# PacificBiosciences/pb-StarPhase

Hardware: AMD Instinct MI355X
Metric: HiFi reads/sec diplotyped (HLA+CYP2D6) (higher is better)
Workload: dtype int32; 1 GPU; BASELINE configs[1] + configs[2] as ONE sample per step: HLA-A/-B 10000 HiFi reads vs IMGT/HLA v0.14.1 (11,199 DNA alleles) + CYP2D6 2000 targeted reads (39 templates), the six configs[2] scenarios in turn; a new sample uploaded every step; reads -> diplotypes; hla_reads=10000, cyp2d6_reads=2000, cyp2d6_lanes=6, hla_lanes=2, cyp2d6_consensus=launch pairs

## Files before the change

### pb-starphase_amd/csrc/sp_api.hip

```cpp
#include "sp_internal.h"
#include <algorithm>
#include <thread>
#include <atomic>
#include <cstring>
#include <new>
#include <unistd.h>

extern "C" {

int32_t sp_abi_version(void) { return SP_ABI_VERSION; }

int32_t sp_device_count(int32_t* count) {
    int n = 0;
    hipError_t e = hipGetDeviceCount(&n);
    if (count) *count = (e == hipSuccess) ? n : 0;
    return e == hipSuccess ? SP_OK : SP_ERR_NO_DEVICE;
}

int32_t sp_ctx_create(int32_t device, void* stream, sp_ctx** out) {
    if (!out) return SP_ERR_INVALID_ARG;
    *out = nullptr;
    static std::atomic<int> effective{-1};
    bool by_library = false;
    if (effective.load() < 0) {
        bool hip_up = false;
        char link[64];
        for (int fd = 0; fd < 1024 && !hip_up; ++fd) {
            char path[64]; std::snprintf(path, sizeof path, "/proc/self/fd/%d", fd);
            const ssize_t k = readlink(path, link, sizeof link - 1);
            if (k > 0) { link[k] = 0; hip_up = std::strcmp(link, "/dev/kfd") == 0; }
        }
        const char* had = std::getenv("GPU_MAX_HW_QUEUES");
        if (!had && !hip_up) { (void)setenv("GPU_MAX_HW_QUEUES", "16", 0); by_library = true; }
        const char* now = std::getenv("GPU_MAX_HW_QUEUES");
        effective.store(now ? std::atoi(now) : (hip_up ? 0 : 4));
    }
    const int hw_queues = effective.load() > 0 ? effective.load() : 4;
    int n = 0;
    if (hipGetDeviceCount(&n) != hipSuccess || n <= 0 || device < 0 || device >= n) return SP_ERR_NO_DEVICE;
    if (hipSetDevice(device) != hipSuccess) return SP_ERR_NO_DEVICE;
    hipDeviceProp_t prop;
    if (hipGetDeviceProperties(&prop, device) != hipSuccess) return SP_ERR_NO_DEVICE;
    if (std::strncmp(prop.gcnArchName, "gfx950", 6) != 0) return SP_ERR_NO_DEVICE;
    sp_ctx* ctx = new (std::nothrow) sp_ctx();
    if (!ctx) return SP_ERR_OUT_OF_MEMORY;
    ctx->device = device;
    ctx->num_cus = prop.multiProcessorCount > 0 ? prop.multiProcessorCount : 256;
    static bool set_here = false;
    if (by_library) set_here = true;
    ctx->hw_queues = hw_queues; ctx->hw_queues_by_library = set_here;
    ctx->hw_queues_effective = effective.load();
    { const char* kc = std::getenv("SP_K8_COMPOUND"); if (kc && *kc) ctx->k8_compound = std::atoi(kc); }
    { const char* ks = std::getenv("SP_K8_SIDE_ORDERS"); if (ks && *ks) ctx->k8_side_orders = std::max(0, std::min(3, std::atoi(ks))); }
    { const char* kp = std::getenv("SP_K8_PERSISTENT"); if (kp && *kp) ctx->k8_persistent = std::atoi(kp); }
    if (effective.load() == 0)
        ctx->warning = "the HIP runtime was initialised before the library's first context and GPU_MAX_HW_QUEUES was not set: the process's streams share the runtime's 4 hardware queues; "
                       "export GPU_MAX_HW_QUEUES=16 (or more) before the process initialises HIP";
    else if (hw_queues < 16)
        ctx->warning = "GPU_MAX_HW_QUEUES=" + std::to_string(hw_queues) + ": the library's streams share " + std::to_string(hw_queues) +
                       " hardware queues; export GPU_MAX_HW_QUEUES=16 (or more) before the process initialises HIP";
    if (stream) { ctx->stream = (hipStream_t)stream; ctx->own_stream = false; }
    else {
        if (hipStreamCreateWithFlags(&ctx->stream, hipStreamNonBlocking) != hipSuccess) { delete ctx; return SP_ERR_HIP; }
        ctx->own_stream = true;
    }
    if (hipEventCreate(&ctx->ev0) != hipSuccess || hipEventCreate(&ctx->ev1) != hipSuccess) { delete ctx; return SP_ERR_HIP; }
    *out = ctx;
    return SP_OK;
}

int32_t sp_ctx_get_info(const sp_ctx* ctx, sp_ctx_info* out) {
    if (!ctx || !out) return SP_ERR_INVALID_ARG;
    std::memset(out, 0, sizeof *out);
    out->device = ctx->device; out->num_cus = ctx->num_cus; out->hw_queues = ctx->hw_queues; out->hw_queues_set_by_library = ctx->hw_queues_by_library ? 1 : 0;
    std::snprintf(out->warning, sizeof out->warning, "%s", ctx->warning.c_str());
    return SP_OK;
}

static int32_t upload_finish(sp_seqset* s);
void sp_ctx_destroy(sp_ctx* ctx) {
    if (!ctx) return;
    for (sp_ctx*& h : ctx->helper) if (h) { sp_ctx_destroy(h); h = nullptr; }
    hipSetDevice(ctx->device);
    if (ctx->uploading) (void)upload_finish(ctx->uploading);
    if (ctx->copy_stream) { hipStreamSynchronize(ctx->copy_stream); hipStreamDestroy(ctx->copy_stream); ctx->copy_stream = nullptr; }
    if (ctx->ctl_stream) { hipStreamSynchronize(ctx->ctl_stream); hipStreamDestroy(ctx->ctl_stream); ctx->ctl_stream = nullptr; }
    if (ctx->ev_fork) hipEventDestroy(ctx->ev_fork);
    if (ctx->ev_join) hipEventDestroy(ctx->ev_join);
    hipStreamSynchronize(ctx->stream);
    for (sp_seqset* s : ctx->live_sets) {
        for (void* p : { (void*)s->d_words, (void*)s->d_nplane, (void*)s->d_word_off, (void*)s->d_len, (void*)s->d_kcode, (void*)s->d_kpos, (void*)s->d_koff }) if (p) ctx->dev_cap.erase(p);
        s->ctx = nullptr;
    }
    for (auto& kv : ctx->dev_cap) (void)hipFree(kv.first);
    if (ctx->scratch) hipFree(ctx->scratch);
    for (auto& kv : ctx->pool) if (kv.second.first) hipFree(kv.second.first);
    for (auto& kv : ctx->host_pool) if (kv.second.first) hipHostFree(kv.second.first);
    sp_profile_flush(ctx);
    for (hipEvent_t e : ctx->prof_free) hipEventDestroy(e);
    if (ctx->ev0) hipEventDestroy(ctx->ev0);
    if (ctx->ev1) hipEventDestroy(ctx->ev1);
    if (ctx->own_stream && ctx->stream) hipStreamDestroy(ctx->stream);
    delete ctx;
}

}
sp_ctx* sp_ctx_helper(sp_ctx* ctx, int i) {
    if (i < 0 || i > 6) return nullptr;
    if (!ctx->helper[i] && sp_ctx_create(ctx->device, nullptr, &ctx->helper[i]) != SP_OK) ctx->helper[i] = nullptr;
    if (ctx->helper[i]) { ctx->helper[i]->profiling = ctx->profiling; ctx->helper[i]->k5_block_pairs = ctx->k5_block_pairs; ctx->helper[i]->k8_persistent = ctx->k8_persistent; ctx->helper[i]->k8_side_orders = ctx->k8_side_orders; ctx->helper[i]->k8_compound = ctx->k8_compound; ctx->helper[i]->k8_side_max_blocks = ctx->k8_side_max_blocks; ctx->helper[i]->mm2_rescore = ctx->mm2_rescore; ctx->helper[i]->profile_rescore_counts = ctx->profile_rescore_counts; ctx->helper[i]->k1_best_n = ctx->k1_best_n; }
    return ctx->helper[i];
}
void sp_profile_merge(sp_ctx* into, sp_ctx* from) {
    sp_profile_flush(from);
    for (auto& kv : from->prof) { ProfileEntry& e = into->prof[kv.first]; e.ms += kv.second.ms; e.launches += kv.second.launches; e.cells += kv.second.cells; }
    from->prof.clear();
}
extern "C" {

int32_t sp_struct_size(const char* name) {
    if (!name) return -1;
#define SP_SZ(T) if (std::strcmp(name, #T) == 0) return (int32_t)sizeof(T);
    SP_SZ(sp_ctx_info)
    SP_SZ(sp_pair)
    SP_SZ(sp_aln)
    SP_SZ(sp_hla_db_desc)
    SP_SZ(sp_hla_realign)
    SP_SZ(sp_k1_seed_hit)
    SP_SZ(sp_hla_best)
    SP_SZ(sp_chain_problem)
    SP_SZ(sp_chain_result)
    SP_SZ(sp_region_hit)
    SP_SZ(sp_cyp_problem)
    SP_SZ(sp_cyp_call)
    SP_SZ(sp_cyp_locus)
    SP_SZ(sp_cyp_gene_def)
    SP_SZ(sp_cyp_config)
    SP_SZ(sp_cyp_db_stats)
    SP_SZ(sp_variant_problem)
    SP_SZ(sp_variant_result)
    SP_SZ(sp_sv_definitions)
    SP_SZ(sp_cons_config)
    SP_SZ(sp_cons_result)
    SP_SZ(sp_cons_problem)
    SP_SZ(sp_cons_output)
    SP_SZ(sp_priority_problem)
    SP_SZ(sp_priority_job)
    SP_SZ(sp_hla_call_config)
    SP_SZ(sp_hla_call)
    SP_SZ(sp_diplotype_settings)
    SP_SZ(sp_sample_inputs)
    SP_SZ(sp_starphase_timing)
    SP_SZ(sp_cyp_read_mapping)
    SP_SZ(sp_database_metadata)
    SP_SZ(sp_database_stats)
    SP_SZ(sp_gene_region)
    SP_SZ(sp_variant_detail)
    SP_SZ(sp_bam_read)
    SP_SZ(sp_affine_opts)
    SP_SZ(sp_affine_aln)
    SP_SZ(sp_k1_seed_info)
    SP_SZ(sp_cyp_region_variants)
    SP_SZ(sp_chain_build_info)
    SP_SZ(sp_variant_gene_stats)
    SP_SZ(sp_vcf_allele)
    SP_SZ(sp_vcf_deletion)
    SP_SZ(sp_mapping_stats)
    SP_SZ(sp_hla_rev_hit)
    SP_SZ(sp_batch_options)
    SP_SZ(sp_starphase_batch_timing)
    SP_SZ(sp_hla_alleles_stats)
    SP_SZ(sp_hla_cfg_mapping)
    SP_SZ(sp_hla_cfg_gene)
    SP_SZ(sp_pileup_col)
    SP_SZ(sp_support_summary)
    SP_SZ(sp_support_entry)
#undef SP_SZ
    return -1;
}

const char* sp_last_error(const sp_ctx* ctx) { return ctx ? ctx->err.c_str() : "null context"; }

int32_t sp_ctx_synchronize(sp_ctx* ctx) {
    if (!ctx) return SP_ERR_INVALID_ARG;
    SP_HIP_CHECK(ctx, hipStreamSynchronize(ctx->stream));
    return SP_OK;
}

int32_t sp_ctx_set_option(sp_ctx* ctx, const char* name, int64_t value) {
    if (!ctx || !name) return SP_ERR_INVALID_ARG;
    if (std::strcmp(name, "hla_split_genes") == 0) { ctx->split_genes = value != 0; return SP_OK; }
    if (std::strcmp(name, "k1_best_n") == 0) { if (value < 0 || value > 8) return sp_fail(ctx, SP_ERR_INVALID_ARG, "sp_ctx_set_option: k1_best_n is 0..8"); ctx->k1_best_n = (int)value; for (sp_ctx* h : ctx->helper) if (h) h->k1_best_n = ctx->k1_best_n; return SP_OK; }
    if (std::strcmp(name, "profile_rescore_counts") == 0) { ctx->profile_rescore_counts = value != 0; for (sp_ctx* h : ctx->helper) if (h) h->profile_rescore_counts = ctx->profile_rescore_counts; return SP_OK; }
    if (std::strcmp(name, "mm2_rescore") == 0) { ctx->mm2_rescore = (int)value; for (sp_ctx* h : ctx->helper) if (h) h->mm2_rescore = ctx->mm2_rescore; return SP_OK; }
    if (std::strcmp(name, "k8_side_orders") == 0) { if (value < 0 || value > 3) return sp_fail(ctx, SP_ERR_INVALID_ARG, "sp_ctx_set_option: k8_side_orders is 0 .. 3"); ctx->k8_side_orders = (int)value; for (sp_ctx* h : ctx->helper) if (h) h->k8_side_orders = ctx->k8_side_orders; return SP_OK; }
    if (std::strcmp(name, "k8_compound") == 0) { ctx->k8_compound = (int)value; for (sp_ctx* h : ctx->helper) if (h) h->k8_compound = ctx->k8_compound; return SP_OK; }
    if (std::strcmp(name, "k8_side_max_blocks") == 0) { if (value < 0) return sp_fail(ctx, SP_ERR_INVALID_ARG, "sp_ctx_set_option: k8_side_max_blocks >= 0"); ctx->k8_side_max_blocks = (int)value; for (sp_ctx* h : ctx->helper) if (h) h->k8_side_max_blocks = ctx->k8_side_max_blocks; return SP_OK; }
    if (std::strcmp(name, "k8_persistent") == 0) { if (value < 0 || value > 2) return sp_fail(ctx, SP_ERR_INVALID_ARG, "sp_ctx_set_option: k8_persistent is 0 (never), 1 (whenever a batch fits) or 2 (the library decides)"); ctx->k8_persistent = (int)value; ctx->k8_persist_backoff = 0; ctx->k8_persist_failures = 0; for (sp_ctx* h : ctx->helper) if (h) h->k8_persistent = ctx->k8_persistent; return SP_OK; }
    if (std::strcmp(name, "cons_retry_ladder") == 0) { ctx->cons_retry_ladder = value != 0; for (sp_ctx* h : ctx->helper) if (h) h->cons_retry_ladder = ctx->cons_retry_ladder; return SP_OK; }
    if (std::strcmp(name, "k5_block_pairs") == 0) { if (value < 0 || value > (1 << 20)) return sp_fail(ctx, SP_ERR_INVALID_ARG, "sp_ctx_set_option: k5_block_pairs is 0..1048576"); ctx->k5_block_pairs = (int)value; for (sp_ctx* h : ctx->helper) if (h) h->k5_block_pairs = ctx->k5_block_pairs; return SP_OK; }
    if (std::strcmp(name, "cyp_cohort_min_group") == 0) { if (value < 1 || value > 64) return sp_fail(ctx, SP_ERR_INVALID_ARG, "sp_ctx_set_option: cyp_cohort_min_group is 1..64"); ctx->cyp_cohort_min_group = (int)value; return SP_OK; }
    if (std::strcmp(name, "cyp_cohort_streams") == 0) { if (value < 1 || value > 8) return sp_fail(ctx, SP_ERR_INVALID_ARG, "sp_ctx_set_option: cyp_cohort_streams is 1..8"); ctx->cyp_cohort_streams = (int)value; return SP_OK; }
    if (std::strcmp(name, "hla_split_streams") == 0) { if (value < 1 || value > 4) return sp_fail(ctx, SP_ERR_INVALID_ARG, "sp_ctx_set_option: hla_split_streams is 1..4"); ctx->split_streams = (int)value; return SP_OK; }
    return sp_fail(ctx, SP_ERR_INVALID_ARG, std::string("sp_ctx_set_option: unknown option ") + name);
}

int32_t sp_profile_reset(sp_ctx* ctx) {
    if (!ctx) return SP_ERR_INVALID_ARG;
    for (sp_ctx* h : ctx->helper) if (h) sp_profile_reset(h);
    sp_profile_flush(ctx); ctx->prof.clear();
    unsigned long long* c = sp_counters(ctx);
    if (c) { hipSetDevice(ctx->device); hipMemsetAsync(c, 0, SPC_N * sizeof(unsigned long long), ctx->stream); }
    return SP_OK;
}

int32_t sp_profile_get(sp_ctx* ctx, const char* kernel, double* total_ms, uint64_t* launches, uint64_t* cells) {
    if (!ctx || !kernel) return SP_ERR_INVALID_ARG;
    sp_profile_flush(ctx);
    for (sp_ctx* h : ctx->helper) if (h) sp_profile_merge(ctx, h);
    static const struct { const char* name; int idx; } counters[] = {
        {"count:k1_cells_active", SPC_K1_ACTIVE}, {"count:k1_cells_executed", SPC_K1_EXECUTED}, {"count:k1_cells_resumed", SPC_K1_RESUMED},
        {"count:k1_cells_bytes", SPC_K1_BYTES}, {"count:cons_launches", SPC_CONS_LAUNCHES}, {"count:cons_columns", SPC_CONS_COLUMNS},
        {"count:dbg0", 6}, {"count:dbg1", 7}, {"count:dbg2", 8}, {"count:dbg3", 9}, {"count:dbg4", 10}, {"count:dbg5", 11}, {"count:dbg6", 12}, {"count:dbg7", 13} };
    for (const auto& c : counters) if (std::strcmp(kernel, c.name) == 0) {
        unsigned long long v = 0; unsigned long long* d = sp_counters(ctx);
        if (d) { hipSetDevice(ctx->device); if (hipMemcpyAsync(&v, d + c.idx, 8, hipMemcpyDeviceToHost, ctx->stream) != hipSuccess || hipStreamSynchronize(ctx->stream) != hipSuccess) return sp_fail(ctx, SP_ERR_HIP, "sp_profile_get: counter read failed"); }
        for (sp_ctx* h : ctx->helper) if (h) {
            unsigned long long hv = 0; unsigned long long* hd = sp_counters(h);
            if (hd && hipMemcpyAsync(&hv, hd + c.idx, 8, hipMemcpyDeviceToHost, h->stream) == hipSuccess && hipStreamSynchronize(h->stream) == hipSuccess) v += hv;
        }
        if (total_ms) *total_ms = 0.0;
        if (launches) *launches = 0;
        if (cells) *cells = v;
        return SP_OK;
    }
    if (std::strcmp(kernel, "pool:device") == 0) {
        uint64_t allocs = ctx->pool_allocs, bytes = ctx->scratch_bytes;
        for (const auto& b : ctx->pool) bytes += b.second.second;
        for (sp_ctx* h : ctx->helper) if (h) { allocs += h->pool_allocs; bytes += h->scratch_bytes; for (const auto& b : h->pool) bytes += b.second.second; }
        if (total_ms) *total_ms = 0.0;
        if (launches) *launches = allocs;
        if (cells) *cells = bytes;
        return SP_OK;
    }
    auto it = ctx->prof.find(kernel);
    ProfileEntry e; if (it != ctx->prof.end()) e = it->second;
    if (total_ms) *total_ms = e.ms;
    if (launches) *launches = e.launches;
    if (cells) *cells = e.cells;
    return SP_OK;
}


struct sp_upload {
    std::thread th;
    int32_t rc = SP_OK; std::string err;
    int format = SP_SEQ_ASCII;
    const uint8_t* src = nullptr; uint64_t src_bytes = 0;
    std::vector<uint64_t> rel;
    uint8_t* d_stage = nullptr; uint64_t* d_off = nullptr; uint32_t* d_flag = nullptr;
    uint8_t* ring = nullptr; size_t chunk = 0; int slots = 0;
    hipEvent_t slot_ev[4] = { nullptr, nullptr, nullptr, nullptr };
    size_t wbytes = 0;
};

static constexpr size_t UPLOAD_CHUNK = (size_t)8 << 20;
static constexpr int UPLOAD_SLOTS = 4;

static void upload_run(sp_seqset* s) {
    sp_upload* u = s->up; sp_ctx* ctx = s->ctx;
    hipStream_t st = ctx->copy_stream;
    auto bad = [&](hipError_t e, const char* what) { if (e != hipSuccess && u->rc == SP_OK) { u->rc = SP_ERR_HIP; u->err = std::string(what) + ": " + hipGetErrorString(e); } return e != hipSuccess; };
    if (bad(hipSetDevice(ctx->device), "hipSetDevice")) return;
    const uint32_t n = s->n;
    bad(hipMemcpyAsync(s->d_word_off, s->h_word_off.data(), ((size_t)n + 1) * sizeof(uint64_t), hipMemcpyHostToDevice, st), "offsets");
    if (n) bad(hipMemcpyAsync(s->d_len, s->h_len.data(), (size_t)n * sizeof(int32_t), hipMemcpyHostToDevice, st), "lengths");
    bad(hipMemsetAsync(s->d_words, 0, u->wbytes, st), "clear");
    if (u->src_bytes && u->rc == SP_OK) {
        bad(hipMemcpyAsync(u->d_off, u->rel.data(), ((size_t)n + 1) * 8, hipMemcpyHostToDevice, st), "staged offsets");
        bad(hipMemsetAsync(u->d_flag, 0, 4, st), "flag");
// ... 423 lines not shown
```

### pb-starphase_amd/csrc/sp_consensus.hip

```cpp
#include "sp_internal.h"
#include <atomic>
#include <cstdlib>
#include "sp_wfa.hip.h"
#include <algorithm>
#include <cstddef>
#include <cstring>
#include <map>
#include <string>

namespace {

constexpr int CB = 64;
constexpr int CH = 32;
#ifndef SP_K8_WAVES
#define SP_K8_WAVES 8
#endif
#ifndef SP_K8_MIN_WAVES
#define SP_K8_MIN_WAVES 4
#endif
constexpr int CWAVES = SP_K8_WAVES;
#ifndef SP_K8_DBG_READS
#define SP_K8_DBG_READS 16384
#endif
#define SP_K8_DBG_LAUNCHES (4194304 / SP_K8_DBG_READS)
#ifndef SP_K8_CW
#define SP_K8_CW 256
#endif
constexpr int CW = SP_K8_CW;
static_assert(CW % 64 == 0 && CW >= 64 && CW <= 512, "window length");
constexpr int CWIN = 512;
constexpr int RWORDS = (2 * CW + 320) / 16;
constexpr int NQ = 56;
constexpr int NWORK = 4;
constexpr int MAXKIDS = 16;
constexpr int CLUSTER = 64;
constexpr int RSLICES = 16;
constexpr int RGROUP = 16;
constexpr int QSV = 2 * (CW + 1) * 5, QSL = 2 * CW * 4, QE = QSV + QSL + 2 * (CW + 1);
enum { F_ACTIVE = 1, F_FINISHED = 2, F_LOST = 4 };
enum { M_NONE = 0, M_INIT = 1, M_WINDOW = 2, M_EXPAND = 3 };

struct CWork {
    int32_t mode, done;
    int32_t node, in_slot;
    int32_t T, n, replay;
    int32_t dual, split_at;
    int32_t go[2];
    int32_t n_kids, pad;
    int32_t pre_go[2];
    int32_t kid_node[MAXKIDS];
    int8_t  kid_base[MAXKIDS][2];
    int8_t  kid_split[MAXKIDS];
    uint8_t spec[2][CW];
};
struct CNode {
    int32_t used, id, complete;
    int32_t T, cur;
    int32_t dual, split_at, stopped[2], len[2];
    int32_t n, a, q;
    int16_t have_out, la_valid;
    int32_t wcap;
    long long cost0;
    long long rest;
    long long rest_out;
    uint32_t ev[2][5];
    int32_t pex_n, pex_L;
    int8_t  pex_kid[MAXKIDS];
    int32_t pad_head[2];
    int32_t dc[CW + 1];
    uint8_t spec[2][CW];
    int32_t pad_[3];
    __device__ __forceinline__ long long cost_at(int j) const { return cost0 + (long long)dc[j]; }
};
constexpr int NODE_HEAD_WORDS = 40, NODE_WORDS = (int)(sizeof(CNode) / 4), NODE_TAPE_WORDS = NODE_WORDS - NODE_HEAD_WORDS;
static_assert(offsetof(CNode, dc) == 4 * NODE_HEAD_WORDS && sizeof(CNode) % 16 == 0, "CNode layout");
struct CSearch {
    int32_t threshold, farthest, next_id, best_node, inflight, max_queue, per_size, wo_constraint;
    int32_t windows, cut_windows, expansions, pops_mod;
    long long pops, best_final;
    long long ticks[4];
    long long step_ticks, gap_ticks, last_end;
    int32_t compound, compound_ok;
    long long gap_ctl_ticks;
    int32_t steps, side_windows, side_expansions, adopted;
#ifdef SP_K8_PF_PROBE
    int32_t pf_win, pf_replay, pf_exp, pf_pad;
    unsigned long long idle_mask;
#endif
};
struct ConsMeta { int32_t e, c0, flags, pad; };
// ... 423 lines not shown
                }
                if (!__ballot(go && nm == 16 && left > 16)) break;
            }
        }, span, lane);
    } else if (span > 0 && !(d.flags & F_FINISHED) && !(et && rv.n <= span + CB)) {
        const int kk = lane - CH;
        dwfa_catchup_t(d, rv.n, [&]() {
            for (;;) {
                bool go = d.H >= 0 && d.H < rv.n && d.H + kk < span;
                if (go) { const int x = rbc(d.H); go = x < 4 && x == ca(d.c0 + d.H + kk); }
                if (!__ballot(go)) break;
                if (go) d.H += 1;
            }
        }, span, lane);
    } else {
        for (int Tl = 1; Tl <= span; ++Tl) {
            if (d.flags & (F_FINISHED | F_LOST)) break;
            dwfa_push_t(d, rv.n, rbc, [&](Dwfa& x, int Tc) {
                const int kk = lane - CH;
                for (;;) {
                    bool go = x.H >= 0 && x.H < rv.n && x.H + kk < Tc;
                    if (go) { const int b = rbc(x.H); go = b < 4 && b == ca(x.c0 + x.H + kk); }
                    if (!__ballot(go)) break;
                    if (go) x.H += 1;
                }
            }, Tl, ca(c0 + Tl - 1), et, lane);
        }
    }
    ACT_T(3);
    return d;
}

constexpr int KID_LA_KIDS = 4, KID_LA = CW / KID_LA_KIDS;
#ifndef SP_K8_KID_W0
#define SP_K8_KID_W0 32
#endif
constexpr int KID_W0 = SP_K8_KID_W0 < KID_LA ? SP_K8_KID_W0 : KID_LA;
#ifndef SP_K8_RAMP
#define SP_K8_RAMP 2
#endif
#ifndef SP_K8_KID_CALM
#define SP_K8_KID_CALM 6
#endif
constexpr int KID_CALM = SP_K8_KID_CALM;
struct UsedWords {
    int used, has_la, a_end, b_end, total;
    __device__ __forceinline__ UsedWords(int mode, int n, int n_kids) {
        used = mode == M_EXPAND ? n_kids : (mode == M_WINDOW ? n + 1 + n_kids : 1);
        has_la = mode != M_EXPAND || n_kids <= KID_LA_KIDS;
        a_end = 2 * used * 5; b_end = a_end + (has_la ? QSL : 0); total = b_end + 2 * used;
    }
    __device__ __forceinline__ int at(int c) const {
        if (c < a_end) { const int i = c / (used * 5), rem = c % (used * 5); return (i * (CW + 1) + rem / 5) * 5 + rem % 5; }
        if (c < b_end) return QSV + (c - a_end);
        const int r = c - b_end;
        return r < used ? QSV + QSL + r : QSV + QSL + (CW + 1) + (r - used);
    }
};
template <class BT> __device__ __forceinline__ uint32_t block_word(const BT& B, size_t blk, int o) {
    constexpr int EV = 2 * (CW + 1), EL = 2 * CW, EC = CW + 1;
    if (o < QSV) { const int e = o / 5, f = o % 5; return f < 4 ? (uint32_t)((B.PV[blk * EV + e] >> (16 * f)) & 0xFFFFull) : B.PE[blk * EV + e]; }
    if (o < QSV + QSL) { const int e = (o - QSV) / 4, f = (o - QSV) % 4; return (uint32_t)((B.PL[blk * EL + e] >> (16 * f)) & 0xFFFFull); }
    if (o < QSV + QSL + EC) return B.PC[blk * EC + (o - QSV - QSL)];
    return B.PR[blk * EC + (o - QSV - QSL - EC)];
}
#ifndef SP_K8_WRAMP0
#define SP_K8_WRAMP0 64
#endif
constexpr int WRAMP0 = SP_K8_WRAMP0;
constexpr int BULK_MARGIN_PLACED = 2;
constexpr int BULK_MARGIN = 8;
#ifndef SP_K8_AUTO_BATCHES
#define SP_K8_AUTO_BATCHES 1
#endif
constexpr int PERSIST_AUTO_BATCHES = SP_K8_AUTO_BATCHES;
#ifndef SP_K8_LIGHT
#define SP_K8_LIGHT 64
#endif
constexpr int PERSIST_LIGHT = SP_K8_LIGHT;
#ifndef SP_K8_DIRECT_BLOCKS
#define SP_K8_DIRECT_BLOCKS (680 * 8 / SP_K8_WAVES)
#endif
constexpr int DIRECT_BLOCKS = SP_K8_DIRECT_BLOCKS;
constexpr int32_t SP_K8_AGAIN = -777;
constexpr int PERSIST_BLOCKS = 128 * 8 / CWAVES;

template <int MAXP> __device__ __forceinline__ int block_problem(const ConsBatchT<MAXP>& B, int block) {
    int pi = 0;
    if constexpr (MAXP == 0) pi = B.block_prob[block];
    else {
#pragma unroll
        for (int i = 1; i < MAXP; ++i) if (i < B.n_prob && block >= B.p[i].first_block) pi = i;
    }
    return pi;
}
template <int MAXP> __device__ __forceinline__ int block_problem(const ConsBatchT<MAXP>& B) { return block_problem<MAXP>(B, (int)blockIdx.x); }

__device__ __forceinline__ size_t state_plane(int node, int slot, int cons) { return (size_t)((node * 2 + slot) * 2 + cons); }

__device__ __forceinline__ int read_cost(const Dwfa& a0, const Dwfa& a1, bool dualrun) {
    int c = -1;
    if (a0.flags & F_ACTIVE) c = a0.e;
    if (dualrun && (a1.flags & F_ACTIVE) && (c < 0 || a1.e < c)) c = a1.e;
    return c < 0 ? 0 : c;
}

template <int MAXP>
__device__ __forceinline__ void cons_step_body(const ConsBatchT<MAXP>& B, const int wrow) {
    __shared__ unsigned long long lv[2][CW + 1];
    __shared__ uint32_t le[2][CW + 1];
    __shared__ unsigned long long ll[2][CW];
    __shared__ uint32_t lc[CW + 1], lr[CW + 1];
    __shared__ uint8_t cwin[2][CWIN + CW];
    __shared__ uint32_t rwin[CWAVES][2][RWORDS + 2];
    __shared__ uint32_t cpk[2][(CWIN + CW) / 16 + 2];
    __shared__ ActScratch act[CWAVES];
    __shared__ CWork wk_s;
    const int pi = block_problem<MAXP>(B);
    const ConsParams P = B.p[pi];
    const bool coh = B.sync != nullptr;
    if (coh) {
        for (int x = threadIdx.x; x < (int)(sizeof(CWork) / 4); x += blockDim.x) ((uint32_t*)&wk_s)[x] = coh_load(((const uint32_t*)P.work) + x);
        __syncthreads();
    }
    const CWork* Wp = coh ? &wk_s : P.work + wrow;
    const int mode = Wp->mode;
    if (P.work->done || mode == M_NONE) return;
    if (wrow > 0 && P.n_blocks > DIRECT_BLOCKS) return;
    if (B.step_t && threadIdx.x == 0) atomicMin(&B.step_t[2 * pi], (unsigned long long)wall_clock64());
    const int lane = threadIdx.x & 63, wave = threadIdx.x >> 6;
    const int T = Wp->T, n = (mode == M_WINDOW || mode == M_EXPAND) ? Wp->n : 0;
    const int pre = mode == M_EXPAND ? n : 0;
    const int node = Wp->node, in_slot = Wp->in_slot;
    const int dual_in = Wp->dual, split_at = Wp->split_at;
    const int go0 = Wp->go[0], go1 = Wp->go[1];
    const int n_kids = (mode == M_EXPAND || mode == M_WINDOW) ? Wp->n_kids : 0;
    const uint8_t* Cn = P.C + (size_t)node * 2 * P.cs;
    for (int x = threadIdx.x; x < 2 * (CW + 1); x += blockDim.x) { (&lv[0][0])[x] = 0; (&le[0][0])[x] = 0; }
    for (int x = threadIdx.x; x < 2 * CW; x += blockDim.x) (&ll[0][0])[x] = 0;
    for (int x = threadIdx.x; x < CW + 1; x += blockDim.x) { lc[x] = 0; lr[x] = 0; }
    const int w0 = T - CWIN;
    for (int x = threadIdx.x; x < 2 * (CWIN + CW); x += blockDim.x) {
        const int i = x / (CWIN + CW), y = x % (CWIN + CW), pos = w0 + y;
        uint8_t v = 0;
        if (pos >= T) v = (pos - T < n) ? Wp->spec[dual_in ? i : 0][pos - T] : 0;
        else if (pos >= 0) v = coh_load((i == 1 && dual_in && pos >= split_at) ? &Cn[(size_t)P.cs + pos] : &Cn[pos]);
        cwin[i][y] = v;
    }
    __syncthreads();
    constexpr int CPW = (CWIN + CW) / 16 + 2;
    for (int x = threadIdx.x; x < 2 * CPW; x += blockDim.x) {
        const int i = x / CPW, w = x % CPW;
        uint32_t word = 0;
        for (int b = 0; b < 16; ++b) { const int y = w * 16 + b; if (y < CWIN + n) word |= (uint32_t)(cwin[i][y] & 3u) << (b << 1); }
        cpk[i][w] = word;
    }
    __syncthreads();
    const size_t plane = (size_t)B.total;
    for (int rr = 0; rr < P.rpw; ++rr) {
        const int r = (((int)blockIdx.x - P.first_block) * CWAVES + wave) * P.rpw + rr;
        if (r >= P.n) break;
        const size_t g = (size_t)P.first + r;
#ifdef SP_K8_TIMING
        const long long wt0 = wall_clock64();
        if (lane == 0) { act[wave].tk[0] = act[wave].tk[1] = act[wave].tk[2] = act[wave].tk[3] = 0; }
#endif
        const ReadInfo ri = B.info[g];
        ReadView rv; rv.w = ri.w; rv.np = ri.np; rv.n = ri.n;
        if (lane == 0) act[wave].staged = nullptr;
        Dwfa d0, d1;
        d0.H = SP_NEG; d0.e = 0; d0.c0 = 0; d0.flags = 0; d1 = d0;
        if (mode == M_INIT) {
            if (ri.off < 0) { d0.flags = F_ACTIVE | ((P.et && rv.n == 0) ? F_FINISHED : 0); d0.H = lane == CH ? 0 : SP_NEG; }
        } else {
            const size_t p0 = state_plane(node, in_slot, 0) * plane + g;
            const ConsMeta m0 = B.meta[p0];
            d0.H = h_load(B.H, p0 * CB + lane); d0.e = m0.e; d0.c0 = m0.c0; d0.flags = m0.flags;
            if (dual_in) {
                const size_t p1 = state_plane(node, in_slot, 1) * plane + g;
                const ConsMeta m1 = B.meta[p1];
                d1.H = h_load(B.H, p1 * CB + lane); d1.e = m1.e; d1.c0 = m1.c0; d1.flags = m1.flags;
            }
        }
        int rbase = 0;
        {
            int lo = 0x7FFFFFFF;
            if (d0.flags & F_ACTIVE) { const int x = T - d0.c0 - CB; lo = x < lo ? x : lo; }
            if (dual_in && (d1.flags & F_ACTIVE)) { const int x = T - d1.c0 - CB; lo = x < lo ? x : lo; }
            if (lo == 0x7FFFFFFF || lo < 0) lo = 0;
            rbase = (lo >> 4) << 4;
            const int w_first = rbase >> 4, w_last = (rv.n + 15) >> 4;
            if (lane < RWORDS + 2) {
                const int w = w_first + lane;
                rwin[wave][0][lane] = w <= w_last + 1 ? rv.w[w] : 0u;
                rwin[wave][1][lane] = (rv.np && w <= w_last + 1) ? rv.np[w] : 0u;
            }
            spw::wave_lds_sync();
        }
        auto rb = [&](int h) -> int {
            const int x = h - rbase;
            if ((unsigned)x < (unsigned)(RWORDS * 16)) {
                const uint32_t sh = (uint32_t)(x & 15) << 1;
                if ((rwin[wave][1][x >> 4] >> sh) & 1u) return 4;
                return (int)((rwin[wave][0][x >> 4] >> sh) & 3u);
            }
            return read_base(rv, h);
        };
        auto vote = [&](const Dwfa& a, const Dwfa& o, bool dualrun, int i, int col, int slot) {
            if (!(a.flags & F_ACTIVE) || (a.flags & (F_FINISHED | F_LOST))) return;
            if (dualrun && (o.flags & F_ACTIVE) && !(o.flags & F_LOST) && o.e < a.e) return;
            const int Tl = col - a.c0, k = lane - CH;
            const bool tip = a.H >= 0 && a.H + k == Tl;
            const int code = (tip && a.H < rv.n) ? rb(a.H) : 5;
            int dc = 0; unsigned long long word = 0;
#pragma unroll
            for (int b = 0; b < 4; ++b) { const bool s = __ballot(code == b) != 0; dc += s; word |= s ? (1ull << (16 * b)) : 0ull; }
            const bool ended = __ballot(tip) != 0 && __ballot(code == 4) == 0;
            if (lane == 0) {
                if (dc) atomicAdd(&lv[i][slot], word * vote_units(dc));
                else if (ended) atomicAdd(&le[i][slot], 12u);
            }
        };
        bool use_pk = mode == M_WINDOW;
        auto extender = [&](const ConsAccess& cacc, int i) {
            return [&cacc, i, &rb, wave, rbase, w0, lane, &use_pk, &rv](Dwfa& d, int Tc) {
                const int k = lane - CH;
                for (;;) {
                    int left = rv.n - d.H; { const int l2 = Tc - (d.H + k); left = l2 < left ? l2 : left; }
                    const bool go = d.H >= 0 && left > 0;
                    int nm = 0; bool more = false;
                    if (go) {
                        const int xr = d.H - rbase, yc = d.c0 + d.H + k - w0;
                        if (use_pk && xr >= 0 && xr < RWORDS * 16 && yc >= 0 && yc < CWIN + CW) {
                            const uint32_t a = __builtin_amdgcn_alignbit(rwin[wave][0][(xr >> 4) + 1], rwin[wave][0][xr >> 4], (uint32_t)(xr & 15) << 1);
                            const uint32_t nn = __builtin_amdgcn_alignbit(rwin[wave][1][(xr >> 4) + 1], rwin[wave][1][xr >> 4], (uint32_t)(xr & 15) << 1);
                            const uint32_t b = __builtin_amdgcn_alignbit(cpk[i][(yc >> 4) + 1], cpk[i][yc >> 4], (uint32_t)(yc & 15) << 1);
                            const uint32_t xo = a ^ b, mm = ((xo | (xo >> 1)) | nn) & 0x55555555u;
                            nm = mm ? (__builtin_ctz(mm) >> 1) : 16;
                            nm = nm < left ? nm : left;
                            more = nm == 16 && left > 16;
                        } else {
                            const int x = rb(d.H);
                            nm = (x < 4 && x == cacc.at(d.c0 + d.H + k)) ? 1 : 0;
// ... 288 lines not shown
                const int kb0 = Wp->kid_base[k][0], kb1 = Wp->kid_base[k][1], ksplit = Wp->kid_split[k];
                if (ksplit) e1 = e0;
                const bool kdual = dual_in || ksplit;
                ConsAccess k0 = ca0, k1 = ca1;
                k0.ov_pos = kb0 >= 0 ? TB : -1; k0.ov_base = kb0;
                k1.ov_pos = kb1 >= 0 ? TB : -1; k1.ov_base = kb1;
                if (ksplit) { k1.i = 0; }
                column(e0, e1, kdual, kb0 >= 0, kb1 >= 0, kb0, kb1, TB + 1, k0, k1);
                if (kb0 >= 0) vote(e0, e1, kdual, 0, TB + 1, s0 + k);
                if (kdual && kb1 >= 0) vote(e1, e0, kdual, 1, TB + 1, s0 + k);
                if (n_kids <= KID_LA_KIDS && (P.n < 256 || (r & 3) == 0)) {
#pragma unroll
                    for (int i = 0; i < 2; ++i) {
                        if (i == 1 && !kdual) continue;
                        if ((i ? kb1 : kb0) < 0) continue;
                        const Dwfa& a = i ? e1 : e0; const Dwfa& o = i ? e0 : e1;
                        if (!(a.flags & F_ACTIVE) || (a.flags & (F_FINISHED | F_LOST))) continue;
                        if (kdual && (o.flags & F_ACTIVE) && !(o.flags & F_LOST) && o.e < a.e) continue;
                        const int Tl = TB + 1 - a.c0, kd = lane - CH;
                        unsigned long long tips = __ballot(a.H >= 0 && a.H + kd == Tl && a.H < rv.n);
                        unsigned long long* const kl = &ll[0][0] + (size_t)(k * 2 + i) * KID_LA;
                        for (int cnt = 0; tips && cnt < 2; ++cnt) {
                            const int tl = __builtin_ctzll(tips); tips &= tips - 1;
                            const int h = __builtin_amdgcn_readlane(a.H, tl);
                            for (int x = lane; x < KID_LA - 1 && h + 1 + x < rv.n; x += SP_WAVE) {
                                const int b = rb(h + 1 + x);
                                if (b < 4) atomicAdd(&kl[x], 1ull << (16 * b));
                            }
                        }
                    }
                }
                const int grow = read_cost(e0, e1, kdual) - base_cost;
                const int len0 = kb0 >= 0 ? TB + 1 : (go0 ? TB : coh_load(&P.nodes[node].len[0]));
                const int len1 = kb1 >= 0 ? TB + 1 : (go1 ? TB : coh_load(&P.nodes[node].len[1]));
                const int extra = final_extra(e0, e1, kdual, len0, len1);
                if (lane == 0) { if (grow) atomicAdd(&lc[s0 + k], (uint32_t)grow); if (extra) atomicAdd(&lr[s0 + k], (uint32_t)extra); }
                const int kn = Wp->kid_node[k];
                store(e0, kn, 0, 0);
                if (kdual) store(e1, kn, 0, 1);
            }
            spw::wave_lds_sync();
        };
        if (mode == M_EXPAND) {
            if (pre > 0) { use_pk = true; win_pass(d0, d1, dual_in != 0, Wp->pre_go[0], Wp->pre_go[1], pre, true); use_pk = false; }
            expand_kids(d0, d1, T + pre, 0);
#ifdef SP_K8_DBG_PARTS
            if (B.dbg && lane == 0 && Wp->pad < SP_K8_DBG_LAUNCHES / 2 && g < SP_K8_DBG_READS) {
                const unsigned long long dt = (unsigned long long)(wall_clock64() - wt0);
                B.dbg[((size_t)Wp->pad * SP_K8_DBG_READS + g) * 2] = (dt > 0xFFFFFF ? 0xFFFFFFull : dt) | ((unsigned long long)(n_kids > 511 ? 511 : n_kids) << 24) | (3ull << 43) | ((unsigned long long)(pre > 511 ? 511 : pre) << 45);
                B.dbg[((size_t)Wp->pad * SP_K8_DBG_READS + g) * 2 + 1] = 0;
            }
#endif
            continue;
        }

        win_pass(d0, d1, dual_in != 0, go0, go1, n, false);
        if (n_kids > 0) {
            use_pk = false;
            if (lane == 0) act[wave].staged = nullptr;
            spw::wave_lds_sync();
            expand_kids(d0, d1, T + n, n + 1);
        }
    }
    __syncthreads();
    const UsedWords uw(mode, n, n_kids);
    if (P.n_blocks <= DIRECT_BLOCKS) {
        const size_t blk = (size_t)P.acc_block + (size_t)wrow;
        for (int x = threadIdx.x; x < 2 * uw.used; x += blockDim.x) {
            const int i = x / uw.used, e = i * (CW + 1) + x % uw.used;
            const unsigned long long v = (&lv[0][0])[e]; const uint32_t w = (&le[0][0])[e];
            if (v) atomicAdd(&B.PV[blk * 2 * (CW + 1) + e], v);
            if (w) atomicAdd(&B.PE[blk * 2 * (CW + 1) + e], w);
        }
        if (uw.has_la) for (int x = threadIdx.x; x < 2 * CW; x += blockDim.x) { const unsigned long long v = (&ll[0][0])[x]; if (v) atomicAdd(&B.PL[blk * 2 * CW + x], v); }
        for (int x = threadIdx.x; x < uw.used; x += blockDim.x) {
            if (lc[x]) atomicAdd(&B.PC[blk * (CW + 1) + x], lc[x]);
            if (lr[x]) atomicAdd(&B.PR[blk * (CW + 1) + x], lr[x]);
        }
        if (B.step_t && threadIdx.x == 0) atomicMax(&B.step_t[2 * pi + 1], (unsigned long long)wall_clock64());
        return;
    }
    for (int x = threadIdx.x; x < 2 * uw.used; x += blockDim.x) {
        const int i = x / uw.used, e = i * (CW + 1) + x % uw.used;
        B.PV[(size_t)blockIdx.x * 2 * (CW + 1) + e] = (&lv[0][0])[e];
        B.PE[(size_t)blockIdx.x * 2 * (CW + 1) + e] = (&le[0][0])[e];
    }
    if (uw.has_la) for (int x = threadIdx.x; x < 2 * CW; x += blockDim.x) B.PL[(size_t)blockIdx.x * 2 * CW + x] = (&ll[0][0])[x];
    for (int x = threadIdx.x; x < uw.used; x += blockDim.x) { B.PC[(size_t)blockIdx.x * (CW + 1) + x] = lc[x]; B.PR[(size_t)blockIdx.x * (CW + 1) + x] = lr[x]; }
    if (B.step_t && threadIdx.x == 0) atomicMax(&B.step_t[2 * pi + 1], (unsigned long long)wall_clock64());
}

template <int MAXP>
__global__ void __launch_bounds__(CWAVES * SP_WAVE, SP_K8_MIN_WAVES) cons_step_kernel(ConsBatchT<MAXP> B) { cons_step_body<MAXP>(B, (int)blockIdx.y); }
template <int MAXP>
__global__ void __launch_bounds__(CWAVES * SP_WAVE, 2) cons_step_wide_kernel(ConsBatchT<MAXP> B) { cons_step_body<MAXP>(B, (int)blockIdx.y); }

template <int MAXP>
__global__ void __launch_bounds__(512) cons_reduce_kernel(ConsBatchT<MAXP> B) {
    const int cluster = (int)blockIdx.x / RSLICES, slice = (int)blockIdx.x % RSLICES;
    int pi = 0;
    if constexpr (MAXP == 0) pi = B.cluster_prob[cluster];
    else {
#pragma unroll
        for (int i = 1; i < MAXP; ++i) if (i < B.n_prob && cluster >= B.p[i].first_cluster) pi = i;
    }
    const ConsParams P = B.p[pi];
    const int mode = P.work->mode;
    if (P.work->done || mode == M_NONE) return;
    const UsedWords uw(mode, mode == M_WINDOW ? P.work->n : 0, mode == M_EXPAND ? P.work->n_kids : 0);
    if (P.n_blocks <= DIRECT_BLOCKS) return;
    const int cl = cluster - P.first_cluster;
    const int members = P.n_blocks - cl * CLUSTER < CLUSTER ? P.n_blocks - cl * CLUSTER : CLUSTER;
    const size_t blk0 = (size_t)P.first_block + (size_t)cl * CLUSTER;
    constexpr int NG = CLUSTER / RGROUP;
    const int per = (uw.total + RSLICES - 1) / RSLICES;
    const int c_lo = slice * per, c_hi = c_lo + per < uw.total ? c_lo + per : uw.total;
    for (int idx = threadIdx.x; idx < (c_hi - c_lo) * NG; idx += blockDim.x) {
        const int o = uw.at(c_lo + idx / NG), m0 = (idx % NG) * RGROUP;
        uint32_t v[RGROUP];
#pragma unroll
        for (int m = 0; m < RGROUP; ++m) v[m] = m0 + m < members ? block_word(B, blk0 + m0 + m, o) : 0u;
        uint32_t sum = 0;
#pragma unroll
        for (int m = 0; m < RGROUP; ++m) sum += v[m];
#pragma unroll
        for (int d = 1; d < NG; d <<= 1) sum += __shfl_xor(sum, d);
        if (idx % NG == 0) B.Q[(size_t)cluster * QE + o] = sum;
    }
}

struct ColVotes { uint32_t w[4], end; };

__device__ __forceinline__ int col_candidates(const uint32_t* w5, int col, int cap, int et, int min_count, double min_af, int out[4]) {
    if (col >= cap) return 0;
    int order[4] = { 0, 1, 2, 3 };
#pragma unroll
    for (int a = 0; a < 4; ++a)
#pragma unroll
        for (int b = a + 1; b < 4; ++b) if (w5[order[b]] > w5[order[a]]) { const int t = order[a]; order[a] = order[b]; order[b] = t; }
    const uint32_t w1 = w5[order[0]], total = w5[0] + w5[1] + w5[2] + w5[3];
    const bool go = et ? w1 > 0 : (total > w5[4] && w1 > 0);
    if (!go) return 0;
    uint32_t need = 12u * (uint32_t)min_count; if (w1 < need) need = w1;
    int n = 0;
    out[n++] = order[0];
#pragma unroll
    for (int a = 1; a < 4; ++a) { const uint32_t w = w5[order[a]]; if (w > 0 && w >= need && (double)w >= min_af * (double)total) out[n++] = order[a]; }
    return n;
}

__device__ __forceinline__ int col_candidates_packed(const uint32_t* w5, int col, int cap, int et, int min_count, double min_af, uint32_t& packed) {
    packed = 0;
    if (col >= cap) return 0;
    uint32_t wa = w5[0], wb = w5[1], wc = w5[2], wd = w5[3]; uint32_t ca = 0, cb = 1, cc = 2, cd = 3;
#define SP_CSW(x, y, cx, cy) if (y > x) { const uint32_t tw_ = x; x = y; y = tw_; const uint32_t tc_ = cx; cx = cy; cy = tc_; }
    SP_CSW(wa, wb, ca, cb) SP_CSW(wa, wc, ca, cc) SP_CSW(wa, wd, ca, cd) SP_CSW(wb, wc, cb, cc) SP_CSW(wb, wd, cb, cd) SP_CSW(wc, wd, cc, cd)
#undef SP_CSW
    const uint32_t total = wa + wb + wc + wd;
    const bool go = et ? wa > 0 : (total > w5[4] && wa > 0);
    if (!go) return 0;
    uint32_t need = 12u * (uint32_t)min_count; if (wa < need) need = wa;
    int n = 1; packed = ca;
    const double floor_w = min_af * (double)total;
    if (wb > 0 && wb >= need && (double)wb >= floor_w) { packed |= cb << (2 * n); ++n; }
    if (wc > 0 && wc >= need && (double)wc >= floor_w) { packed |= cc << (2 * n); ++n; }
    if (wd > 0 && wd >= need && (double)wd >= floor_w) { packed |= cd << (2 * n); ++n; }
    return n;
}

template <int MAXP>
__device__ __forceinline__ void cons_control_body(const ConsBatchT<MAXP>& B) {
    extern __shared__ uint8_t proc[];
    __shared__ uint32_t acc[QE];
    uint32_t (*sv)[CW + 1][5] = reinterpret_cast<uint32_t (*)[CW + 1][5]>(acc);
    uint32_t (*sl)[CW][4] = reinterpret_cast<uint32_t (*)[CW][4]>(acc + QSV);
    uint32_t* sc = acc + QSV + QSL; uint32_t* sr = sc + (CW + 1);
    __shared__ CNode nh[NQ];
    __shared__ CWork wks[NWORK];
    __shared__ CSearch ss;
    __shared__ int copy_from[NWORK], copy_len[NWORK], need_la[NWORK], replay_of[NWORK];
    struct KidCopy { int from, T, n, nk, dual; int8_t node[4], b0[4], b1[4], sp[4]; uint8_t spec[2][CW]; };
    static_assert(KID_LA_KIDS <= 4, "KidCopy");
    __shared__ KidCopy kcopy[NWORK];
    const int pi = blockIdx.x;
    const ConsParams P = B.p[pi];
    const int tid = threadIdx.x;
    const bool coh = B.sync != nullptr;
    const int nside = (coh || P.n_blocks > DIRECT_BLOCKS) ? 0 : (B.nside < NWORK - 1 ? B.nside : NWORK - 1);
    const int n_orders = 1 + nside;
    CWork& wk = wks[0];
    const long long tk0 = wall_clock64();
    for (int x = tid; x < NQ * NODE_HEAD_WORDS; x += blockDim.x)
        ((uint32_t*)&nh[x / NODE_HEAD_WORDS])[x % NODE_HEAD_WORDS] = ((const uint32_t*)&P.nodes[x / NODE_HEAD_WORDS])[x % NODE_HEAD_WORDS];
    for (int x = tid; x < n_orders * (int)(sizeof(CWork) / 4); x += blockDim.x) ((uint32_t*)wks)[x] = ((const uint32_t*)P.work)[x];
    for (int x = tid; x < (int)(sizeof(CSearch) / 4); x += blockDim.x) ((uint32_t*)&ss)[x] = ((const uint32_t*)P.srch)[x];
    const int proc_words = (P.cap + 2 + 3) / 4;
    for (int x = tid; x < proc_words; x += blockDim.x) ((uint32_t*)proc)[x] = ((const uint32_t*)P.processed)[x];
    for (int x = tid; x < QE; x += blockDim.x) acc[x] = 0;
    if (tid < NWORK) { copy_from[tid] = -1; copy_len[tid] = 0; need_la[tid] = -1; replay_of[tid] = -1; kcopy[tid].nk = 0; if (tid >= n_orders) wks[tid].mode = M_NONE; }
    __syncthreads();
    if (wk.done) return;
    auto tape_word_used = [](const CNode& x, int w) {
        if (!x.used) return false;
        if (w == 0) return true;
        if (x.n <= 0) return false;
        if (w < CW + 1) return w <= x.n;
        const int sw = w - (CW + 1);
        return sw < 2 * (CW / 4) && (sw % (CW / 4)) * 4 < x.n;
    };
    for (int x = tid; x < NQ * NODE_TAPE_WORDS; x += blockDim.x) {
        const int k = x / NODE_TAPE_WORDS, w = x % NODE_TAPE_WORDS;
        if (tape_word_used(nh[k], w)) ((uint32_t*)&nh[k])[NODE_HEAD_WORDS + w] = ((const uint32_t*)&P.nodes[k])[NODE_HEAD_WORDS + w];
    }
    auto load_votes = [&](const int w) {
        const int mode_in = wks[w].mode, n_in = (mode_in == M_WINDOW || mode_in == M_EXPAND) ? wks[w].n : 0;
        if (mode_in == M_NONE) return;
        const UsedWords uw(mode_in, n_in, wks[w].n_kids);
        if (P.n_blocks <= DIRECT_BLOCKS) {
            const int u = uw.used, ev = 2 * u, el = uw.has_la ? 2 * CW : 0, E = ev + ev + el + u + u;
            const size_t blk = (size_t)P.acc_block + (size_t)w;
            for (int c = tid; c < E; c += blockDim.x) {
                if (c < ev || (c >= 2 * ev && c < 2 * ev + el)) {
                    const bool exact = c < ev;
                    const int e = exact ? (c / u) * (CW + 1) + c % u : c - 2 * ev;
                    unsigned long long* src = exact ? B.PV + blk * 2 * (CW + 1) + e : B.PL + blk * 2 * CW + e;
                    const unsigned long long sum = coh ? __hip_atomic_exchange(src, 0ull, __ATOMIC_RELAXED, __HIP_MEMORY_SCOPE_AGENT) : *src;
                    if (sum) {
                        if (!coh) *src = 0ull;
                        uint32_t* dst = exact ? acc + e * 5 : acc + QSV + e * 4;
#pragma unroll
                        for (int f = 0; f < 4; ++f) dst[f] = (uint32_t)((sum >> (16 * f)) & 0xFFFFull);
                    }
                } else {
                    uint32_t* src; uint32_t* dst;
                    if (c < 2 * ev) { const int cc = c - ev, e = (cc / u) * (CW + 1) + cc % u; src = B.PE + blk * 2 * (CW + 1) + e; dst = acc + e * 5 + 4; }
                    else if (c < 2 * ev + el + u) { const int e = c - 2 * ev - el; src = B.PC + blk * (CW + 1) + e; dst = acc + QSV + QSL + e; }
                    else { const int e = c - 2 * ev - el - u; src = B.PR + blk * (CW + 1) + e; dst = acc + QSV + QSL + (CW + 1) + e; }
                    const uint32_t sum = coh ? __hip_atomic_exchange(src, 0u, __ATOMIC_RELAXED, __HIP_MEMORY_SCOPE_AGENT) : *src;
                    if (sum) { if (!coh) *src = 0u; *dst = sum; }
                }
            }
        } else {
            const int parts = P.n_clusters;
            for (int c = tid; c < uw.total; c += blockDim.x) {
                const int o = uw.at(c);
                uint32_t sum = 0;
                for (int c0 = 0; c0 < parts; c0 += 8) {
                    uint32_t v[8];
#pragma unroll
                    for (int q = 0; q < 8; ++q) v[q] = c0 + q < parts ? B.Q[(size_t)(P.first_cluster + c0 + q) * QE + o] : 0u;
#pragma unroll
                    for (int q = 0; q < 8; ++q) sum += v[q];
                }
                acc[o] = sum;
            }
        }
    };
    const int lane = tid & (SP_WAVE - 1);
    auto cands = [&](const uint32_t* w5, int col, int out[4]) { return col_candidates(w5, col, P.cap, P.et, P.min_count, P.min_af, out); };
    auto node_free = [&](int k) {
        const int np = nh[k].pex_n;
        for (int j = 0; j < np; ++j) { CNode& c = nh[nh[k].pex_kid[j]]; c.used = 0; c.complete = 0; }
        nh[k].pex_n = 0; nh[k].used = 0; nh[k].complete = 0;
    };
    uint8_t* Cb = P.C;
    int la_fresh = -1;
    auto trim_queue = [&]() {
// ... 536 lines not shown
                if (lane == 0 && W.n == bcol) {
                    Plan fp; fp.nc0 = bn0; fp.nc1 = bn1; fp.cd0 = bc0; fp.cd1 = bc1;
                    const int kids = !W.dual ? bn0 + (P.allow_dual ? bn0 * (bn0 - 1) / 2 : 0) : (bn0 ? bn0 : 1) * (bn1 ? bn1 : 1);
                    unsigned long long fm = free_mask;
                    int made = 0;
                    for (int k = 0; k < kids && fm; ++k) {
                        int b0, b1, sp;
                        kid_of(fp, W.dual, k, b0, b1, sp);
                        const int kn = __builtin_ctzll(fm); fm &= fm - 1;
                        nh[kn].used = 2; nh[kn].complete = 0; nh[kn].pex_n = 0;
                        W.kid_node[made] = kn; W.kid_base[made][0] = (int8_t)b0; W.kid_base[made][1] = (int8_t)b1; W.kid_split[made] = (int8_t)sp;
                        ++made;
                    }
                    W.n_kids = made;
                    ss.compound += 1;
                }
                spw::wave_lds_sync();
            }
        }
    }
    __syncthreads();
    for (int w = 0; w < n_orders; ++w) {
        if (copy_from[w] < 0) continue;
        const CWork& W = wks[w];
        const int cfrom = copy_from[w], clen = copy_len[w];
        for (int k = 0; k < W.n_kids; ++k) {
            const int kn = W.kid_node[k];
            const bool split = W.kid_split[k] != 0;
            for (int i = 0; i < 2; ++i) {
                if (i == 1 && !(W.dual || split)) continue;
                const uint4* src = reinterpret_cast<const uint4*>(P.C + ((size_t)cfrom * 2 + ((i == 1 && split) ? 0 : i)) * P.cs);
                uint8_t* dst = P.C + ((size_t)kn * 2 + i) * P.cs;
                const int whole = clen >> 4, tail = clen & 15;
                for (int y = tid; y < whole + (tail ? 1 : 0); y += blockDim.x) {
                    uint4 v;
                    if (coh) {
                        const unsigned long long* s8 = reinterpret_cast<const unsigned long long*>(src + y);
                        const unsigned long long lo = coh_load(s8), hi = coh_load(s8 + 1);
                        v.x = (uint32_t)lo; v.y = (uint32_t)(lo >> 32); v.z = (uint32_t)hi; v.w = (uint32_t)(hi >> 32);
                    } else v = src[y];
                    if (y == whole && W.kid_base[k][i] >= 0) reinterpret_cast<uint8_t*>(&v)[tail] = (uint8_t)W.kid_base[k][i];
                    if (coh) {
                        unsigned long long* d8 = reinterpret_cast<unsigned long long*>(reinterpret_cast<uint4*>(dst) + y);
                        coh_store(d8, (unsigned long long)v.x | ((unsigned long long)v.y << 32)); coh_store(d8 + 1, (unsigned long long)v.z | ((unsigned long long)v.w << 32));
                    } else reinterpret_cast<uint4*>(dst)[y] = v;
                }
                if (tid == 0 && tail == 0 && W.kid_base[k][i] >= 0) put(&dst[clen], (uint8_t)W.kid_base[k][i], coh);
            }
        }
    }
    if (tid == 0) {
        const long long tk4 = wall_clock64(); ss.ticks[0] += tk1 - tk0; ss.ticks[1] += tk2 - tk1; ss.ticks[2] += tk3 - tk2; ss.ticks[3] += tk4 - tk3;
        if (B.step_t) {
            const long long st0 = (long long)coh_load(&B.step_t[2 * pi]), st1 = (long long)coh_load(&B.step_t[2 * pi + 1]);
            if (st1 > 0 && st0 <= st1) {
                ss.step_ticks += st1 - st0;
                if (ss.last_end > 0 && st0 >= ss.last_end) ss.gap_ticks += st0 - ss.last_end;
                if (tk0 >= st1) { ss.gap_ticks += tk0 - st1; ss.gap_ctl_ticks += tk0 - st1; }
            }
            put(&B.step_t[2 * pi], ~0ull, coh); put(&B.step_t[2 * pi + 1], 0ull, coh);
            ss.last_end = tk4;
        }
    }
#ifdef SP_K8_SEARCH_TICKS
    if (tid == 0) { ss.ticks[0] += 100 * ts_iters - (tk1 - tk0); ss.ticks[1] += ts_pick - (tk2 - tk1); ss.ticks[3] += ts_block - (wall_clock64() - tk3); }
#endif
    __syncthreads();
    for (int x = tid; x < NQ * NODE_HEAD_WORDS; x += blockDim.x)
        put(&((uint32_t*)&P.nodes[x / NODE_HEAD_WORDS])[x % NODE_HEAD_WORDS], ((const uint32_t*)&nh[x / NODE_HEAD_WORDS])[x % NODE_HEAD_WORDS], coh);
    for (int x = tid; x < NQ * NODE_TAPE_WORDS; x += blockDim.x) {
        const int k = x / NODE_TAPE_WORDS, w = x % NODE_TAPE_WORDS;
        if (tape_word_used(nh[k], w)) ((uint32_t*)&P.nodes[k])[NODE_HEAD_WORDS + w] = ((const uint32_t*)&nh[k])[NODE_HEAD_WORDS + w];
    }
    for (int x = tid; x < n_orders * (int)(sizeof(CWork) / 4); x += blockDim.x) put(&((uint32_t*)P.work)[x], ((const uint32_t*)wks)[x], coh);
    for (int x = tid; x < (int)(sizeof(CSearch) / 4); x += blockDim.x) ((uint32_t*)P.srch)[x] = ((const uint32_t*)&ss)[x];
    for (int x = tid; x < proc_words; x += blockDim.x) ((uint32_t*)P.processed)[x] = ((const uint32_t*)proc)[x];
    if (tid == 0 && B.prog) {
        __hip_atomic_store(B.prog + 2 * pi, (uint32_t)wk.pad, __ATOMIC_RELAXED, __HIP_MEMORY_SCOPE_SYSTEM);
        if (wk.done) __hip_atomic_store(B.prog + 2 * pi + 1, 1u, __ATOMIC_RELAXED, __HIP_MEMORY_SCOPE_SYSTEM);
    }
}

template <int MAXP>
__global__ void __launch_bounds__(1024) cons_control_kernel(ConsBatchT<MAXP> B) { cons_control_body<MAXP>(B); }

constexpr long long PERSIST_TIMEOUT = 400000000ll;
constexpr double PERSIST_READY_S = 0.5;
__device__ __forceinline__ bool persist_wait(const uint32_t* word, uint32_t at_least, uint32_t* abort_word) {
    const long long t0 = wall_clock64();
    for (uint32_t spins = 1;; ++spins) {
        if (__hip_atomic_load(word, __ATOMIC_RELAXED, __HIP_MEMORY_SCOPE_AGENT) >= at_least) return true;
        __builtin_amdgcn_s_sleep(1);
        if ((spins & 63u) == 0) {
            if (__hip_atomic_load(abort_word, __ATOMIC_RELAXED, __HIP_MEMORY_SCOPE_AGENT)) return false;
            if (wall_clock64() - t0 > PERSIST_TIMEOUT) { __hip_atomic_store(abort_word, 1u, __ATOMIC_RELAXED, __HIP_MEMORY_SCOPE_AGENT); return false; }
        }
    }
}

template <int MAXP>
__global__ void __launch_bounds__(CWAVES * SP_WAVE, SP_K8_MIN_WAVES) cons_step_persist_kernel(ConsBatchT<MAXP> B) {
    __shared__ int go_on;
    const int pi = block_problem<MAXP>(B);
    uint32_t* sy = B.sync + 4 * pi; uint32_t* abort_word = B.sync + 4 * B.n_prob;
    for (uint32_t k = 1;; ++k) {
        if (threadIdx.x == 0) go_on = persist_wait(sy + 0, k - 1, abort_word) ? 1 : 0;
        __syncthreads();
        if (!go_on) break;
        if (coh_load(&B.p[pi].work->done)) break;
        cons_step_body<MAXP>(B, 0);
        asm volatile("s_waitcnt vmcnt(0)" ::: "memory");
        __syncthreads();
        if (threadIdx.x == 0) __hip_atomic_fetch_add(sy + 1, 1u, __ATOMIC_RELAXED, __HIP_MEMORY_SCOPE_AGENT);
    }
}

template <int MAXP>
__global__ void __launch_bounds__(1024) cons_control_persist_kernel(ConsBatchT<MAXP> B) {
    __shared__ int go_on;
    const int pi = blockIdx.x;
    const uint32_t nb = (uint32_t)B.p[pi].n_blocks;
    uint32_t* sy = B.sync + 4 * pi; uint32_t* abort_word = B.sync + 4 * B.n_prob;
    if (threadIdx.x == 0 && B.ready) __hip_atomic_fetch_add(B.ready, 1u, __ATOMIC_RELAXED, __HIP_MEMORY_SCOPE_SYSTEM);
    for (uint32_t k = 1;; ++k) {
        if (threadIdx.x == 0) {
            go_on = persist_wait(sy + 1, nb * k, abort_word) ? 1 : 0;
            if (go_on && k > B.step_cap) { __hip_atomic_store(abort_word, 2u, __ATOMIC_RELAXED, __HIP_MEMORY_SCOPE_AGENT); go_on = 0; }
        }
        __syncthreads();
        if (!go_on) break;
        __builtin_amdgcn_fence(__ATOMIC_ACQUIRE, "agent");
        cons_control_body<MAXP>(B);
        asm volatile("s_waitcnt vmcnt(0)" ::: "memory");
        __syncthreads();
        const bool done = coh_load(&B.p[pi].work->done) != 0;
        if (threadIdx.x == 0) __hip_atomic_store(sy + 0, k, __ATOMIC_RELAXED, __HIP_MEMORY_SCOPE_AGENT);
        if (done) break;
    }
    if (threadIdx.x == 0 && B.prog) {
        const uint32_t ab = __hip_atomic_load(abort_word, __ATOMIC_RELAXED, __HIP_MEMORY_SCOPE_AGENT);
        if (ab) __hip_atomic_store(B.prog + 2 * pi + 1, 1u + ab, __ATOMIC_RELAXED, __HIP_MEMORY_SCOPE_SYSTEM);
    }
}

__global__ void cons_setup_kernel(ConsSetup S, ReadInfo* __restrict__ info) {
    const int r = blockIdx.x * blockDim.x + threadIdx.x;
    if (r >= S.n) return;
    const uint32_t rid = S.idx ? S.idx[r] : (uint32_t)r;
    ReadInfo ri;
    ri.w = S.reads.words + S.reads.word_off[rid];
    ri.np = S.reads.nplane ? S.reads.nplane + S.reads.word_off[rid] : nullptr;
    ri.n = S.reads.len[rid]; ri.off0 = S.offsets ? S.offsets[r] : -1; ri.off = ri.off0 < 0 ? -1 : ri.off0 + max(0, min(S.cmp_len, ri.n)); ri.pad = 0;
    info[S.first + r] = ri;
}

__global__ void cons_setup_many_kernel(const ConsSetup* __restrict__ S, int n_prob, int total, ReadInfo* __restrict__ info) {
    const int t = blockIdx.x * blockDim.x + threadIdx.x;
    if (t >= total) return;
    int lo = 0, hi = n_prob - 1;
    while (lo < hi) { const int mid = (lo + hi + 1) >> 1; if (S[mid].first <= t) lo = mid; else hi = mid - 1; }
    while (lo + 1 < n_prob && S[lo].n == 0 && S[lo + 1].first <= t) ++lo;
    const ConsSetup& q = S[lo];
    const int r = t - q.first;
    if (r < 0 || r >= q.n) return;
    const uint32_t rid = q.idx ? q.idx[r] : (uint32_t)r;
    ReadInfo ri;
    ri.w = q.reads.words + q.reads.word_off[rid];
    ri.np = q.reads.nplane ? q.reads.nplane + q.reads.word_off[rid] : nullptr;
    ri.n = q.reads.len[rid]; ri.off0 = q.offsets ? q.offsets[r] : -1; ri.off = ri.off0 < 0 ? -1 : ri.off0 + max(0, min(q.cmp_len, ri.n)); ri.pad = 0;
    info[t] = ri;
}

template <int MAXP>
__global__ void __launch_bounds__(SP_WAVE) cons_finalize_kernel(ConsBatchT<MAXP> B, uint8_t* is_cons1, int32_t* score1, int32_t* score2) {
    const int vblock = (int)blockIdx.x / CWAVES, wave = (int)blockIdx.x % CWAVES;
    const int pi = block_problem<MAXP>(B, vblock);
    const ConsParams P = B.p[pi];
    const int lane = threadIdx.x;
    const int best = P.srch->best_node;
    const size_t plane = (size_t)B.total;
    if (vblock == P.first_block && wave == 0) {
        for (int x = threadIdx.x; x < (int)(sizeof(CSearch) / 4); x += blockDim.x) ((uint32_t*)P.out_srch)[x] = ((const uint32_t*)P.srch)[x];
        if (threadIdx.x == 0) {
            ConsRes r; r.best = best; r.dual = 0; r.split_at = -1; r.len1 = r.len2 = 0; r.pad = 0;
            if (best >= 0) { const CNode* x = P.nodes + best; r.dual = x->dual; r.split_at = x->split_at; r.len1 = x->len[0]; r.len2 = x->dual ? x->len[1] : 0; }
            *P.out_res = r;
        }
        if (best >= 0) {
            const uint8_t* src = P.C + (size_t)best * 2 * P.cs;
#pragma unroll
            for (int i = 0; i < 2; ++i) {
                const uint32_t* s4 = reinterpret_cast<const uint32_t*>(src + (size_t)i * P.cs);
                uint8_t* dst = P.out_cons + (size_t)i * P.cap;
                for (int x = (int)threadIdx.x * 4; x < P.cap; x += (int)blockDim.x * 4) {
                    const uint32_t w = s4[x >> 2];
#pragma unroll
                    for (int q = 0; q < 4; ++q) if (x + q < P.cap) dst[x + q] = (uint8_t)(w >> (8 * q));
                }
            }
        }
    }
    for (int rr = 0; rr < P.rpw; ++rr) {
        const int r = ((vblock - P.first_block) * CWAVES + wave) * P.rpw + rr;
        if (r >= P.n) break;
        const size_t g = (size_t)P.first + r;
        int sc[2] = { -1, -1 };
        if (best >= 0) {
            const CNode* x = P.nodes + best;
            const int n = B.info[g].n, cur = x->cur, dual = x->dual;
#pragma unroll
            for (int i = 0; i < 2; ++i) {
                if (i == 1 && !dual) continue;
                const size_t p = state_plane(best, cur, i) * plane + g;
                const ConsMeta m = B.meta[p];
                if (!(m.flags & F_ACTIVE) || (m.flags & F_LOST)) continue;
                int e = m.e;
                if (!P.et) {
                    const int h = h_load(B.H, p * CB + lane), k = lane - CH;
                    int rest = (h >= 0 && h + k == x->len[i] - m.c0) ? n - h : (1 << 30);
#pragma unroll
                    for (int o = 32; o > 0; o >>= 1) { const int other = __shfl_xor(rest, o); rest = other < rest ? other : rest; }
                    if (rest < (1 << 30)) e += rest;
                }
                sc[i] = e;
            }
        }
        if (lane == 0) {
            score1[g] = sc[0]; score2[g] = sc[1];
            is_cons1[g] = !(sc[1] >= 0 && (sc[0] < 0 || sc[1] < sc[0]));
        }
    }
}

}

constexpr int PERSIST_MAX_BATCHES = 4;
struct PersistLease {
    int device = -1, taken = 0;
    static std::atomic<int>& used(int device) { static std::atomic<int> u[64]; return u[device & 63]; }
    static std::atomic<int>& batches(int device) { static std::atomic<int> b[64]; return b[device & 63]; }
    bool take(int dev, int budget, int want, int max_batches) {
        if (batches(dev).fetch_add(1) >= max_batches) { batches(dev).fetch_sub(1); return false; }
        std::atomic<int>& u = used(dev);
        int cur = u.load();
        while (cur + want <= budget) if (u.compare_exchange_weak(cur, cur + want)) { device = dev; taken = want; return true; }
        batches(dev).fetch_sub(1);
        return false;
    }
    void give_back() { if (taken) { used(device).fetch_sub(taken); batches(device).fetch_sub(1); taken = 0; } }
    ~PersistLease() { give_back(); }
};

template <int MAXP>
static int32_t run_chunk(sp_ctx* ctx, uint32_t n_prob, const sp_cons_problem* probs, sp_cons_output* outs) {
    hipStream_t st = ctx->stream;
    HostMarks hm(ctx);
    ConsBatchT<MAXP> B; std::memset(&B, 0, sizeof B);
    B.n_prob = (int)n_prob;
    std::vector<ConsParams> hp(n_prob);
    std::vector<int> block_prob, cluster_prob;
    std::vector<ConsSetup> setup(n_prob);
    std::vector<uint32_t> h_idx; std::vector<int32_t> h_off;
    std::vector<size_t> idx_at(n_prob), off_at(n_prob), c_at(n_prob), proc_at(n_prob);
    size_t total = 0, c_bytes = 0, proc_bytes = 0; int max_cap = 0, n_blocks = 0, n_clusters = 0;
    std::vector<int> expect(n_prob, 0);
    PersistLease lease;
    int persist_rpw = 0;
    int nside = std::max(0, std::min(ctx->k8_side_orders, NWORK - 1));
    {
        uint64_t nb_all = 0;
        for (uint32_t p = 0; p < n_prob; ++p) nb_all += ((probs[p].read_idx ? probs[p].n : probs[p].reads->n) + CWAVES - 1) / CWAVES;
        if (nb_all * CWAVES > (uint64_t)ctx->k8_side_max_blocks * 8) nside = 0;
    }
    struct InFlight {
        int dev; bool cand; int others = 0;
        static std::atomic<int>& count(int d) { static std::atomic<int> c[64]; return c[d & 63]; }
        static std::atomic<int>& cands(int d) { static std::atomic<int> c[64]; return c[d & 63]; }
        static std::atomic<long long>& overlap_ns(int d) { static std::atomic<long long> t[64]; return t[d & 63]; }
        static long long now_ns() { return std::chrono::duration_cast<std::chrono::nanoseconds>(std::chrono::steady_clock::now().time_since_epoch()).count(); }
        bool recent_overlap = false;
        InFlight(int d, bool candidate) : dev(d), cand(candidate) {
            others = count(dev).fetch_add(1);
            const long long t = now_ns();
            if (cand && cands(dev).fetch_add(1) > 0) overlap_ns(dev).store(t);
            const long long last = overlap_ns(dev).load();
            recent_overlap = last != 0 && t - last < 1000000000ll;
        }
        ~InFlight() { count(dev).fetch_sub(1); if (cand) cands(dev).fetch_sub(1); }
    } in_flight(ctx->device, n_prob > 0 && n_prob <= 8 && [&] { uint64_t f = 2 * (uint64_t)n_prob; for (uint32_t p = 0; p < n_prob; ++p) f += ((probs[p].read_idx ? probs[p].n : probs[p].reads->n) + CWAVES - 1) / CWAVES; return f > (uint64_t)PERSIST_LIGHT; }());
    uint64_t footprint = 2 * (uint64_t)n_prob;
    for (uint32_t p = 0; p < n_prob; ++p) footprint += ((probs[p].read_idx ? probs[p].n : probs[p].reads->n) + CWAVES - 1) / CWAVES;
    const bool light = footprint <= (uint64_t)PERSIST_LIGHT;
    const bool persist_wanted = ctx->k8_persistent == 1 || (ctx->k8_persistent == 2 && n_prob <= 8 && ctx->hw_queues_effective >= 16 && ctx->k8_persist_failures < 3 &&
                                                            !in_flight.recent_overlap && light);
    if (ctx->k8_persist_backoff > 0) --ctx->k8_persist_backoff;
    else if (persist_wanted && n_prob > 0) {
        bool small = true;
        for (uint32_t p = 0; p < n_prob; ++p) {
            const uint32_t n = probs[p].read_idx ? probs[p].n : probs[p].reads->n;
            const uint32_t nb = (n + CWAVES - 1) / CWAVES;
            small = small && nb <= (uint32_t)PERSIST_BLOCKS;
        }
        constexpr int WG_PER_CU = SP_K8_MIN_WAVES * 4 / CWAVES;
        int budget = WG_PER_CU * std::max(0, ctx->num_cus - 32); const int ctl = 2 * (int)n_prob;
        { const char* e = std::getenv("SP_K8_BUDGET"); if (e && *e) budget = std::atoi(e); }
        if (small && ctl < budget) {
            for (int scale = 1; scale <= 4 && !persist_rpw; ++scale) {
                uint64_t nb = 0;
                for (uint32_t p = 0; p < n_prob; ++p) { const uint32_t n = probs[p].read_idx ? probs[p].n : probs[p].reads->n; nb += (n + CWAVES * scale - 1) / (CWAVES * scale); }
                if ((int64_t)nb + ctl <= budget && lease.take(ctx->device, budget, (int)nb + ctl, (ctx->k8_persistent == 2 && !light) ? PERSIST_AUTO_BATCHES : PERSIST_MAX_BATCHES)) persist_rpw = scale;
                else if ((int64_t)nb + ctl <= budget) break;
            }
        }
    }
    for (uint32_t p = 0; p < n_prob; ++p) {
        const sp_cons_problem& q = probs[p];
        const uint32_t n = q.read_idx ? q.n : q.reads->n;
        ConsParams& P = hp[p];
        P.n = (int)n; P.cap = (int)outs[p].cap - 1;
        P.cs = (std::max(P.cap, 1) + 1 + 15) & ~15;
        P.first = (int)total; P.first_block = n_blocks;
        P.min_count = q.cfg.min_count; P.delta = q.cfg.dual_max_ed_delta; P.et = q.cfg.allow_early_termination != 0; P.allow_dual = q.cfg.allow_dual != 0;
        P.window = q.cfg.offset_window; P.cmp_len = q.cfg.offset_compare_length; P.min_af = q.cfg.min_af;
        P.rpw = persist_rpw ? persist_rpw : n > 65536 ? 4 : n > 32768 ? 2 : 1;
        const uint32_t per_block = (uint32_t)(CWAVES * P.rpw);
        const uint32_t nb = (n + per_block - 1) / per_block;
        P.n_blocks = (int)nb;
        P.first_cluster = n_clusters; P.n_clusters = (int)((nb + CLUSTER - 1) / CLUSTER);
        n_clusters += P.n_clusters;
        n_blocks += (int)nb;
        if (MAXP == 0) { block_prob.insert(block_prob.end(), nb, (int)p); cluster_prob.insert(cluster_prob.end(), (size_t)P.n_clusters, (int)p); }
        setup[p].reads = q.reads->view(); setup[p].n = (int)n; setup[p].first = (int)total;
        total += (size_t)nb * per_block;
        idx_at[p] = h_idx.size(); if (q.read_idx) h_idx.insert(h_idx.end(), q.read_idx, q.read_idx + n);
        off_at[p] = h_off.size(); if (q.offsets) h_off.insert(h_off.end(), q.offsets, q.offsets + n);
        c_at[p] = c_bytes; c_bytes += (size_t)NQ * 2 * (size_t)P.cs;
        proc_at[p] = proc_bytes; proc_bytes += ((size_t)std::max(P.cap, 1) + 2 + 15) & ~(size_t)15;
        max_cap = std::max(max_cap, P.cap);
        int reach = 0;
        for (uint32_t i = 0; i < n; ++i) {
            const uint32_t r = q.read_idx ? q.read_idx[i] : i;
            const int o = q.offsets && q.offsets[i] > 0 ? q.offsets[i] : 0;
            reach = std::max(reach, o + (r < q.reads->h_len.size() ? q.reads->h_len[r] : P.cap));
        }
        expect[p] = std::min(P.cap, reach);
    }
    if (n_blocks == 0) return SP_OK;
    const size_t planes = (size_t)NQ * 4;
    size_t in_bytes = 0, out_bytes = 0, zero_bytes = 0;
    auto place = [](size_t& total_bytes, size_t bytes) { const size_t at = (total_bytes + 15) & ~(size_t)15; total_bytes = at + bytes; return at; };
    const size_t in_idx = place(in_bytes, sizeof(uint32_t) * h_idx.size()), in_off = place(in_bytes, sizeof(int32_t) * h_off.size());
    const size_t in_work = place(in_bytes, sizeof(CWork) * NWORK * n_prob), in_srch = place(in_bytes, sizeof(CSearch) * n_prob);
    const size_t in_probs = place(in_bytes, MAXP == 0 ? sizeof(ConsParams) * n_prob : 0), in_bp = place(in_bytes, sizeof(int) * block_prob.size());
    const size_t in_cp = place(in_bytes, sizeof(int) * cluster_prob.size());
    const size_t in_setup = place(in_bytes, n_prob > 8 ? sizeof(ConsSetup) * n_prob : 0);
    const size_t out_srch = place(out_bytes, sizeof(CSearch) * n_prob), out_res = place(out_bytes, sizeof(ConsRes) * n_prob);
    const size_t out_is1 = place(out_bytes, total), out_sc = place(out_bytes, sizeof(int32_t) * 2 * total);
    std::vector<size_t> out_cons(n_prob);
    for (uint32_t p = 0; p < n_prob; ++p) out_cons[p] = place(out_bytes, (size_t)2 * std::max(hp[p].cap, 1));
    const size_t zero_nodes = place(zero_bytes, sizeof(CNode) * NQ * n_prob), zero_proc = place(zero_bytes, proc_bytes), zero_info = place(zero_bytes, sizeof(ReadInfo) * total), zero_memo = place(zero_bytes, sizeof(PlaceMemo) * 2 * total * (size_t)(1 + nside));
    const size_t zero_sync = place(zero_bytes, sizeof(uint32_t) * (4 * (size_t)n_prob + 4));
    uint8_t* d_in = (uint8_t*)sp_pool(ctx, "cons_in", in_bytes + 16); uint8_t* h_in = (uint8_t*)sp_host_pool(ctx, "cons_in", in_bytes + 16);
    uint8_t* d_out = (uint8_t*)sp_pool(ctx, "cons_out", out_bytes + 16); uint8_t* h_out = (uint8_t*)sp_host_pool(ctx, "cons_out", out_bytes + 16);
    uint8_t* d_zero = (uint8_t*)sp_pool(ctx, "cons_zero", zero_bytes + 16);
    if (!d_in || !h_in || !d_out || !h_out || !d_zero) return sp_fail(ctx, SP_ERR_OUT_OF_MEMORY, "sp_consensus staging");
    uint32_t* d_idx = (uint32_t*)(d_in + in_idx); int32_t* d_off = (int32_t*)(d_in + in_off);
    uint8_t* d_C = (uint8_t*)sp_pool(ctx, "cons_C", c_bytes);
    CWork* d_work = (CWork*)(d_in + in_work);
    CSearch* d_srch = (CSearch*)(d_in + in_srch);
    CNode* d_nodes = (CNode*)(d_zero + zero_nodes);
    uint32_t* d_la = (uint32_t*)sp_pool(ctx, "cons_la", sizeof(uint32_t) * (size_t)NQ * 2 * CW * 4 * n_prob);
    uint8_t* d_proc = d_zero + zero_proc;
    ReadInfo* d_info = (ReadInfo*)(d_zero + zero_info);
    B.memo = (PlaceMemo*)(d_zero + zero_memo);
    B.sync = persist_rpw ? (uint32_t*)(d_zero + zero_sync) : nullptr;
    B.info = d_info; B.total = (int)total;
// ... 69 lines not shown
        SP_HIP_CHECK(ctx, hipMemsetAsync(B.PL + nb * 2 * CW, 0, sizeof(unsigned long long) * np * 2 * CW, st));
        SP_HIP_CHECK(ctx, hipMemsetAsync(B.PC + nb * (CW + 1), 0, sizeof(uint32_t) * np * (CW + 1), st));
        SP_HIP_CHECK(ctx, hipMemsetAsync(B.PR + nb * (CW + 1), 0, sizeof(uint32_t) * np * (CW + 1), st));
    }
    if (n_prob > 8) hipLaunchKernelGGL(cons_setup_many_kernel, dim3((unsigned)((total + 255) / 256)), dim3(256), 0, st, (const ConsSetup*)(d_in + in_setup), (int)n_prob, (int)total, d_info);
    else for (uint32_t p = 0; p < n_prob; ++p)
        if (setup[p].n) hipLaunchKernelGGL(cons_setup_kernel, dim3((setup[p].n + 255) / 256), dim3(256), 0, st, setup[p], d_info);

    B.nside = persist_rpw ? 0 : nside;
    B.k8_compound = ctx->k8_compound;
    const dim3 grid((uint32_t)n_blocks, (uint32_t)(1 + B.nside)), block(CWAVES * SP_WAVE);
    const bool one_round = n_blocks <= (ctx->num_cus + ctx->num_cus / 4) * (8 / CWAVES);
    size_t proc_lds = ((size_t)max_cap + 2 + 15) & ~(size_t)15;
    {
        hipFuncAttributes fa;
        SP_HIP_CHECK(ctx, hipFuncGetAttributes(&fa, (const void*)cons_control_kernel<MAXP>));
        if (fa.sharedSizeBytes + proc_lds > 160 * 1024) return sp_fail(ctx, SP_ERR_TOO_LONG, "sp_consensus: cap must stay below ~65,000");
    }
    SP_HIP_CHECK(ctx, hipFuncSetAttribute((const void*)cons_control_kernel<MAXP>, hipFuncAttributeMaxDynamicSharedMemorySize, (int)proc_lds));
    uint64_t pairs = 0;
    bool persist_ran = false;
    hm.mark("host:k8_prologue");
    double t_launch = 0.0;
    {
        ProfScope ps(ctx, "cons_steps", total);
        const uint64_t limit = (uint64_t)64 * (uint64_t)(max_cap + 2) + 1024;
        const uint32_t ahead = 3;
        bool need_reduce = false;
        for (uint32_t p = 0; p < n_prob; ++p) need_reduce = need_reduce || hp[p].n_blocks > DIRECT_BLOCKS;
        volatile uint32_t* prog = h_prog;
        bool finished = false;
        if (persist_rpw) {
            if (!ctx->ctl_stream && hipStreamCreateWithFlags(&ctx->ctl_stream, hipStreamNonBlocking) != hipSuccess) return sp_fail(ctx, SP_ERR_HIP, "sp_consensus: control stream");
            if (!ctx->ev_fork && (hipEventCreateWithFlags(&ctx->ev_fork, hipEventDisableTiming) != hipSuccess || hipEventCreateWithFlags(&ctx->ev_join, hipEventDisableTiming) != hipSuccess))
                return sp_fail(ctx, SP_ERR_HIP, "sp_consensus: events");
            SP_HIP_CHECK(ctx, hipFuncSetAttribute((const void*)cons_control_persist_kernel<MAXP>, hipFuncAttributeMaxDynamicSharedMemorySize, (int)proc_lds));
            SP_HIP_CHECK(ctx, hipEventRecord(ctx->ev_fork, st));
            SP_HIP_CHECK(ctx, hipStreamWaitEvent(ctx->ctl_stream, ctx->ev_fork, 0));
            uint32_t* h_ready = (uint32_t*)sp_host_pool(ctx, "cons_ready", 64);
            if (!h_ready) return sp_fail(ctx, SP_ERR_OUT_OF_MEMORY, "sp_consensus ready word");
            *(volatile uint32_t*)h_ready = 0;
            { void* dp = nullptr; SP_HIP_CHECK(ctx, hipHostGetDevicePointer(&dp, h_ready, 0)); B.ready = (uint32_t*)dp; }
            B.step_cap = (uint32_t)std::min<uint64_t>(limit, 0xFFFFFFFFull);
            auto drain = [&]() { (void)hipStreamSynchronize(ctx->ctl_stream); (void)hipStreamSynchronize(st); };
            hipLaunchKernelGGL(cons_control_persist_kernel<MAXP>, dim3(n_prob), dim3(1024), proc_lds, ctx->ctl_stream, B);
            bool all_ready = true;
            {
                const auto t_wait = std::chrono::steady_clock::now();
                const bool forced = std::getenv("SP_K8_FORCE_READY_TIMEOUT") != nullptr;
                while (forced || *(volatile uint32_t*)h_ready < n_prob) {
                    __builtin_ia32_pause();
                    if (forced || std::chrono::duration<double>(std::chrono::steady_clock::now() - t_wait).count() > PERSIST_READY_S) { all_ready = false; break; }
                }
            }
            if (all_ready) {
                hipLaunchKernelGGL(cons_step_persist_kernel<MAXP>, dim3((uint32_t)n_blocks), block, 0, st, B);
                const hipError_t e1 = hipGetLastError();
                const hipError_t e2 = e1 == hipSuccess ? hipEventRecord(ctx->ev_join, ctx->ctl_stream) : e1;
                const hipError_t e3 = e2 == hipSuccess ? hipStreamWaitEvent(st, ctx->ev_join, 0) : e2;
                if (e3 != hipSuccess) {
                    const uint32_t one = 1;
                    if (!ctx->copy_stream) (void)hipStreamCreateWithFlags(&ctx->copy_stream, hipStreamNonBlocking);
                    if (ctx->copy_stream) { (void)hipMemcpyAsync(B.sync + 4 * n_prob, &one, 4, hipMemcpyHostToDevice, ctx->copy_stream); (void)hipStreamSynchronize(ctx->copy_stream); }
                    drain();
                    return sp_fail(ctx, SP_ERR_HIP, std::string("sp_consensus: persistent launch: ") + hipGetErrorString(e3));
                }
                finished = true; persist_ran = true;
            } else {
                const uint32_t one = 1;
                if (!ctx->copy_stream && hipStreamCreateWithFlags(&ctx->copy_stream, hipStreamNonBlocking) != hipSuccess) { drain(); return sp_fail(ctx, SP_ERR_HIP, "sp_consensus: copy stream"); }
                (void)hipMemcpyAsync(B.sync + 4 * n_prob, &one, 4, hipMemcpyHostToDevice, ctx->copy_stream);
                (void)hipStreamSynchronize(ctx->copy_stream);
                (void)hipStreamSynchronize(ctx->ctl_stream);
                lease.give_back();
                ctx->k8_persist_failures += 1; ctx->k8_persist_backoff = 64;
                ctx->warning = "persistent consensus kernels: the control workgroups of a batch found no free CUs within " + std::to_string(PERSIST_READY_S) +
                               " s (another process on this device?): the batch ran launch by launch, and so will the next 64";
                (void)hipMemsetAsync(B.sync, 0, sizeof(uint32_t) * (4 * (size_t)n_prob + 1), st);
                std::memset(h_prog, 0, sizeof(uint32_t) * 2 * n_prob);
                B.sync = nullptr; B.ready = nullptr;
                persist_rpw = 0;
            }
        }
        while (!finished) {
            const auto tl0 = std::chrono::steady_clock::now();
            if (one_round) hipLaunchKernelGGL(cons_step_wide_kernel<MAXP>, grid, block, 0, st, B);
            else hipLaunchKernelGGL(cons_step_kernel<MAXP>, grid, block, 0, st, B);
            if (need_reduce) hipLaunchKernelGGL(cons_reduce_kernel<MAXP>, dim3((uint32_t)n_clusters * RSLICES), dim3(512), 0, st, B);
            hipLaunchKernelGGL(cons_control_kernel<MAXP>, dim3(n_prob), dim3(1024), proc_lds, st, B);
            t_launch += std::chrono::duration<double, std::milli>(std::chrono::steady_clock::now() - tl0).count();
            ++pairs;
            uint64_t spins = 0;
            for (;;) {
                bool all = true; uint32_t slowest = 0xFFFFFFFFu;
                for (uint32_t p = 0; p < n_prob; ++p) if (!prog[2 * p + 1]) { all = false; const uint32_t v = prog[2 * p]; slowest = v < slowest ? v : slowest; }
                if (all) { finished = true; break; }
                if (pairs - slowest <= ahead) break;
                __builtin_ia32_pause();
                if ((++spins & 0xFFFFF) == 0) {
                    const hipError_t q = hipStreamQuery(st);
                    if (q != hipSuccess && q != hipErrorNotReady) return sp_fail(ctx, SP_ERR_HIP, std::string("sp_consensus: ") + hipGetErrorString(q));
                    if (q == hipSuccess) {
                        bool all2 = true; uint32_t slow2 = 0xFFFFFFFFu;
                        for (uint32_t p = 0; p < n_prob; ++p) if (!prog[2 * p + 1]) { all2 = false; const uint32_t v = prog[2 * p]; slow2 = v < slow2 ? v : slow2; }
                        if (all2) { finished = true; break; }
                        if (pairs - slow2 <= ahead) break;
                        return sp_fail(ctx, SP_ERR_HIP, "sp_consensus: the device stopped reporting progress");
                    }
                }
            }
            if (!finished && pairs >= limit) return sp_fail(ctx, SP_ERR_HIP, "sp_consensus: the search did not finish");
        }
    }
#define SP_K8_CHECK(expr) do { const hipError_t e_ = (expr); if (e_ != hipSuccess) { if (persist_ran) { (void)hipStreamSynchronize(ctx->ctl_stream); (void)hipStreamSynchronize(st); } \
        return sp_fail(ctx, SP_ERR_HIP, std::string(#expr) + ": " + hipGetErrorString(e_)); } } while (0)
    SP_K8_CHECK(hipGetLastError());
    hm.mark("host:k8_loop");
    if (ctx->profiling) { auto& e = ctx->prof["host:k8_launch"]; e.ms += t_launch; e.launches += (uint32_t)(2 * pairs); }
    hipLaunchKernelGGL(cons_finalize_kernel<MAXP>, dim3((uint32_t)n_blocks * CWAVES), dim3(SP_WAVE), 0, st, B, d_is1, d_sc, d_sc + total);
    SP_K8_CHECK(hipMemcpyAsync(h_out, d_out, out_bytes, hipMemcpyDeviceToHost, st));
    const uint8_t* h_is1 = h_out + out_is1; const int32_t* h_sc = (const int32_t*)(h_out + out_sc); const ConsRes* h_res = (const ConsRes*)(h_out + out_res);
    SP_K8_CHECK(hipStreamSynchronize(st));
    SP_K8_CHECK(hipGetLastError());
#undef SP_K8_CHECK
    lease.give_back();
    if (persist_ran) {
        for (uint32_t p = 0; p < n_prob; ++p) {
            if (h_prog[2 * p + 1] == 2u) {
                ctx->k8_persist_failures += 1; ctx->k8_persist_backoff = 64;
                if (ctx->k8_persistent == 2) {
                    ctx->warning = "persistent consensus kernels: the kernels of a batch waited for each other for more than four seconds (another process on this device?): the batch ran "
                                   "again launch by launch, and so will the next 64";
                    return SP_K8_AGAIN;
                }
                return sp_fail(ctx, SP_ERR_HIP, "sp_consensus: the persistent kernels of a batch waited for each other for more than four seconds and gave up");
            }
            if (h_prog[2 * p + 1] == 3u) return sp_fail(ctx, SP_ERR_HIP, "sp_consensus: the search did not finish");
            pairs = std::max<uint64_t>(pairs, h_prog[2 * p]);
        }
        ctx->prof["cons_persistent_batches"].cells += 1;
    }
    hm.mark("host:k8_result_wait");
#ifdef SP_K8_TIMING
    if (std::getenv("SP_K8_DUMP")) {
        std::vector<unsigned long long> h((size_t)SP_K8_DBG_LAUNCHES * SP_K8_DBG_READS);
        (void)hipMemcpy(h.data(), B.dbg, h.size() * 8, hipMemcpyDeviceToHost);
        FILE* f = std::fopen(std::getenv("SP_K8_DUMP"), "ab");
        if (f) { const unsigned long long tot = total; std::fwrite(&tot, 8, 1, f); std::fwrite(h.data(), 8, h.size(), f); std::fclose(f); }
    }
#endif
    {
        uint64_t cut = 0, ex = 0, pops = 0;
        for (uint32_t p = 0; p < n_prob; ++p) { cut += (uint64_t)h_srch[p].cut_windows; ex += (uint64_t)h_srch[p].expansions; pops += (uint64_t)h_srch[p].pops; }
        ctx->prof["cons_windows"].cells += pairs; ctx->prof["cons_windows"].launches += 3 * pairs;
        ctx->prof["cons_cut_windows"].cells += cut; ctx->prof["cons_expansions"].cells += ex; ctx->prof["cons_columns"].cells += pops;
        for (uint32_t p = 0; p < n_prob; ++p) {
            ctx->prof["cons_side_windows"].cells += (uint64_t)h_srch[p].side_windows; ctx->prof["cons_side_expansions"].cells += (uint64_t)h_srch[p].side_expansions;
            ctx->prof["cons_adopted"].cells += (uint64_t)h_srch[p].adopted;
            ctx->prof["cons_compound"].cells += (uint64_t)h_srch[p].compound; ctx->prof["cons_compound_ok"].cells += (uint64_t)h_srch[p].compound_ok;
        }
#ifdef SP_K8_PF_PROBE
        {
            uint64_t c0 = 0, c1 = 0, c2 = 0;
            for (uint32_t p = 0; p < n_prob; ++p) {
                const uint64_t st = (uint64_t)h_srch[p].windows + (uint64_t)h_srch[p].expansions, w = (uint64_t)h_srch[p].pf_win + (uint64_t)h_srch[p].pf_replay, e = (uint64_t)h_srch[p].pf_exp;
                c0 = std::max(c0, st); c1 = std::max(c1, st - w); c2 = std::max(c2, st - w - e);
                ctx->prof["cons_pf_win"].cells += (uint64_t)h_srch[p].pf_win; ctx->prof["cons_pf_replay"].cells += (uint64_t)h_srch[p].pf_replay; ctx->prof["cons_pf_exp"].cells += e;
                ctx->prof["cons_all_windows"].cells += (uint64_t)h_srch[p].windows;
            }
            ctx->prof["cons_pf_chain"].cells += c0; ctx->prof["cons_pf_chain_win"].cells += c1; ctx->prof["cons_pf_chain_all"].cells += c2;
        }
#endif
        static const char* tick_names[4] = { "cons_ticks_reduce", "cons_ticks_result", "cons_ticks_search", "cons_ticks_tail" };
        for (int k = 0; k < 4; ++k) { long long m = 0; for (uint32_t p = 0; p < n_prob; ++p) m = std::max(m, h_srch[p].ticks[k]); ctx->prof[tick_names[k]].cells += (uint64_t)m; }
        if (B.step_t) {
            long long best = -1; uint32_t bp = 0;
            for (uint32_t p = 0; p < n_prob; ++p) {
                const long long tot = h_srch[p].step_ticks + h_srch[p].gap_ticks + h_srch[p].ticks[0] + h_srch[p].ticks[1] + h_srch[p].ticks[2] + h_srch[p].ticks[3];
                if (tot > best) { best = tot; bp = p; }
            }
            ctx->prof["cons_path_step_ticks"].cells += (uint64_t)h_srch[bp].step_ticks; ctx->prof["cons_path_gap_ticks"].cells += (uint64_t)h_srch[bp].gap_ticks; ctx->prof["cons_path_gap_ctl_ticks"].cells += (uint64_t)h_srch[bp].gap_ctl_ticks;
            ctx->prof["cons_path_control_ticks"].cells += (uint64_t)(h_srch[bp].ticks[0] + h_srch[bp].ticks[1] + h_srch[bp].ticks[2] + h_srch[bp].ticks[3]);
            ctx->prof["cons_path_steps"].cells += (uint64_t)h_srch[bp].steps;
        }
    }
    static const char dec[4] = { 'A', 'C', 'G', 'T' };
    int32_t rc = SP_OK;
    for (uint32_t p = 0; p < n_prob; ++p) {
        const ConsParams& P = hp[p]; sp_cons_output& o = outs[p];
        const ConsRes& res = h_res[p];
        const int best = res.best, len1 = res.len1, len2 = res.len2, dual = res.dual, split_at = res.split_at;
        if (best >= 0) {
            const uint8_t* c = h_out + out_cons[p];
            for (int x2 = 0; x2 < len1; ++x2) o.cons1[x2] = dec[c[x2] & 3];
            for (int x2 = 0; x2 < len2; ++x2) o.cons2[x2] = dec[(x2 < split_at ? c[x2] : c[(size_t)P.cap + x2]) & 3];
        }
        o.cons1[len1] = '\0'; o.cons2[len2] = '\0';
        for (int r = 0; r < P.n; ++r) { o.is_cons1[r] = h_is1[P.first + r]; o.score1[r] = h_sc[P.first + r]; o.score2[r] = h_sc[total + P.first + r]; }
        o.result.is_dual = dual; o.result.len1 = len1; o.result.len2 = len2; o.result.split_at = split_at;
        o.result.gave_up = best < 0 ? 1 : 0; o.result.best_total = 1; o.result.split_w2 = 0; o.result.split_total = 1;
        o.result.nodes_expanded = h_srch[p].pops;
        if (len1 >= P.cap || len2 >= P.cap) { o.status = SP_ERR_CAPACITY; rc = SP_ERR_CAPACITY; }
    }
    if (rc != SP_OK) sp_fail(ctx, rc, "sp_consensus: a consensus reached cap");
    hm.mark("host:k8_epilogue");
    return rc;
}

static int32_t run_batch(sp_ctx* ctx, uint32_t n_prob, const sp_cons_problem* probs, sp_cons_output* outs) {
    for (uint32_t p = 0; p < n_prob; ++p) {
        const sp_cons_problem& q = probs[p]; sp_cons_output& o = outs[p];
        if (!q.reads || !o.cons1 || !o.cons2 || o.cap == 0 || !o.is_cons1 || !o.score1 || !o.score2) return sp_fail(ctx, SP_ERR_INVALID_ARG, "sp_consensus: null argument");
        if (q.cfg.offset_compare_length > 128 || q.cfg.offset_compare_length < 0 || q.cfg.offset_window < 0 || q.cfg.min_count < 0 ||
            (q.cfg.offset_compare_length > 64 && q.cfg.offset_window + q.cfg.offset_compare_length > ACT_CONS))
            return sp_fail(ctx, SP_ERR_INVALID_ARG, "sp_consensus: offset_compare_length must be in [0, 128] (in [0, 64] when offset_window + offset_compare_length exceeds 512)");
        if (o.cap >= (1u << 22)) return sp_fail(ctx, SP_ERR_TOO_LONG, "sp_consensus: cap must be below 4,194,304");
        if (q.reads->max_len >= 65535) return sp_fail(ctx, SP_ERR_TOO_LONG, "sp_consensus: sequences must be shorter than 65,535 bases");
        std::memset(&o.result, 0, sizeof o.result); o.result.split_at = -1; o.result.best_total = 1; o.status = SP_OK;
        o.cons1[0] = o.cons2[0] = '\0';
        const uint32_t n = q.read_idx ? q.n : q.reads->n;
        if (q.read_idx) for (uint32_t i = 0; i < n; ++i) if (q.read_idx[i] >= q.reads->n) return sp_fail(ctx, SP_ERR_INVALID_ARG, "sp_consensus: read index out of range");
    }
    SP_HIP_CHECK(ctx, hipSetDevice(ctx->device));
    int32_t rc = SP_OK;
    const uint32_t big = 4096;
    for (uint32_t at = 0; at < n_prob; at += big) {
        const uint32_t k = std::min<uint32_t>(big, n_prob - at);
        auto run = [&]() { return k <= 4 ? run_chunk<4>(ctx, k, probs + at, outs + at) : k <= 8 ? run_chunk<8>(ctx, k, probs + at, outs + at)
                                  : k <= CMAXP ? run_chunk<CMAXP>(ctx, k, probs + at, outs + at) : run_chunk<0>(ctx, k, probs + at, outs + at); };
        int32_t e = run();
        if (e == SP_K8_AGAIN) e = run();
        if (e != SP_OK && e != SP_ERR_CAPACITY) return e;
        if (e != SP_OK) rc = e;
    }
    return rc;
}

extern "C" {

int32_t sp_consensus_batch(sp_ctx* ctx, uint32_t n_problems, const sp_cons_problem* problems, sp_cons_output* outputs) {
    if (!ctx) return SP_ERR_INVALID_ARG;
    if (n_problems == 0) return SP_OK;
    if (!problems || !outputs) return sp_fail(ctx, SP_ERR_INVALID_ARG, "sp_consensus_batch: null argument");
    return run_batch(ctx, n_problems, problems, outputs);
}

int32_t sp_consensus_dual_batch(sp_ctx* ctx, uint32_t n_problems, const sp_cons_problem* problems, sp_cons_output* outputs) {
    if (!ctx) return SP_ERR_INVALID_ARG;
    if (n_problems == 0) return SP_OK;
    if (!problems || !outputs) return sp_fail(ctx, SP_ERR_INVALID_ARG, "sp_consensus_dual_batch: null argument");
    std::vector<sp_cons_problem> pr(problems, problems + n_problems);
    for (auto& q : pr) q.cfg.allow_dual = 1;
    return run_batch(ctx, n_problems, pr.data(), outputs);
}

int32_t sp_consensus(sp_ctx* ctx, const sp_seqset* reads, const uint32_t* read_idx, uint32_t n, const int32_t* offsets,
                     const sp_cons_config* cfg, char* cons1, char* cons2, uint32_t cap,
                     uint8_t* is_cons1, int32_t* score1, int32_t* score2, sp_cons_result* result) {
    if (!ctx) return SP_ERR_INVALID_ARG;
    if (!reads || !cfg || !result) return sp_fail(ctx, SP_ERR_INVALID_ARG, "sp_consensus: null argument");
    sp_cons_problem q; q.reads = reads; q.read_idx = read_idx; q.n = n; q.offsets = offsets; q.cfg = *cfg;
    sp_cons_output o; std::memset(&o, 0, sizeof o);
    o.cons1 = cons1; o.cons2 = cons2; o.cap = cap; o.is_cons1 = is_cons1; o.score1 = score1; o.score2 = score2;
    const int32_t rc = run_batch(ctx, 1, &q, &o);
    *result = o.result;
    return rc;
}

int32_t sp_consensus_dual(sp_ctx* ctx, const sp_seqset* reads, const uint32_t* read_idx, uint32_t n, const int32_t* offsets,
                          const sp_cons_config* cfg, char* cons1, char* cons2, uint32_t cap,
                          uint8_t* is_cons1, int32_t* score1, int32_t* score2, sp_cons_result* result) {
    if (!ctx) return SP_ERR_INVALID_ARG;
    if (!reads || !cfg || !result) return sp_fail(ctx, SP_ERR_INVALID_ARG, "sp_consensus_dual: null argument");
    sp_cons_problem q; q.reads = reads; q.read_idx = read_idx; q.n = n; q.offsets = offsets; q.cfg = *cfg;
    sp_cons_output o; std::memset(&o, 0, sizeof o);
    o.cons1 = cons1; o.cons2 = cons2; o.cap = cap; o.is_cons1 = is_cons1; o.score1 = score1; o.score2 = score2;
    const int32_t rc = sp_consensus_dual_batch(ctx, 1, &q, &o);
    *result = o.result;
    return rc;
}

int32_t sp_consensus_priority_many(sp_ctx* ctx, uint32_t n_jobs, sp_priority_job* jobs) {
    if (!ctx) return SP_ERR_INVALID_ARG;
    if (n_jobs && !jobs) return sp_fail(ctx, SP_ERR_INVALID_ARG, "sp_consensus_priority_many: null argument");
    struct Item { std::vector<uint32_t> members; uint32_t level; std::string key; int retry = 0; std::vector<std::string> kept; std::vector<uint8_t> have; };
    struct JobState { std::vector<Item> work, done; int half = 0; bool live = false; };
    static const double retry_min_af[4] = { 0.15, 0.20, 0.30, 0.40 };
    std::vector<JobState> S(n_jobs);
    for (uint32_t j = 0; j < n_jobs; ++j) {
        sp_priority_job& J = jobs[j];
        J.status = SP_OK; J.gave_up = 0;
        const sp_priority_problem* pr = J.problem;
        if (!pr || !J.n_groups || !J.group_of || !J.cons || !pr->levels || pr->n_levels == 0 || J.cap < 2) { J.status = SP_ERR_INVALID_ARG; continue; }
        bool ok = true;
        for (uint32_t l = 0; l < pr->n_levels; ++l) if (!pr->levels[l] || pr->levels[l]->n != pr->n) ok = false;
        if (!ok) { J.status = SP_ERR_INVALID_ARG; continue; }
        *J.n_groups = 0;
        if (pr->n == 0) continue;
        S[j].half = pr->cfg.offset_window / 2; S[j].live = true;
        std::map<int32_t, std::vector<uint32_t>> by_seed;
        for (uint32_t r = 0; r < pr->n; ++r) by_seed[pr->seeds ? (pr->seeds[r] < 0 ? -1 : pr->seeds[r]) : -1].push_back(r);
        uint32_t ord = 0;
        for (auto& kv : by_seed) { Item it; it.members = kv.second; it.level = 0; it.key = std::string(1, (char)('a' + std::min<uint32_t>(ord, 25))) + std::to_string(ord); ++ord; S[j].work.push_back(std::move(it)); }
    }
    auto rebased = [&](uint32_t j, const std::vector<uint32_t>& m, uint32_t level, std::vector<int32_t>& out) -> bool {
        const sp_priority_problem* pr = jobs[j].problem;
        const int32_t* src = pr->offsets ? pr->offsets[level] : nullptr;
        if (!src) return false;
        int64_t mn = INT64_MAX;
        for (uint32_t r : m) mn = std::min<int64_t>(mn, src[r] < 0 ? 0 : src[r]);
        out.resize(m.size());
// ... 115 lines not shown
```

### pb-starphase_amd/csrc/sp_hla_call.hip

```cpp
#include "sp_internal.h"
#include <thread>
#include <system_error>
#include <algorithm>
#include <cstring>

namespace {

constexpr int SEG_WAVES = 4;
constexpr int HPC_WAVES = 2;
constexpr int HPC_MAX = 32768;

__global__ void __launch_bounds__(SEG_WAVES * SP_WAVE) seg_slice_kernel(SeqSetView reads, const uint32_t* __restrict__ idx, const int32_t* __restrict__ start,
                                                                        const int32_t* __restrict__ len, const uint64_t* __restrict__ word_off, int n,
                                                                        uint32_t* __restrict__ out_words, uint32_t* __restrict__ out_nplane) {
    const int lane = threadIdx.x & 63, s = blockIdx.x * SEG_WAVES + (threadIdx.x >> 6);
    if (s >= n) return;
    const uint32_t r = idx[s];
    const uint32_t* src = reads.words + reads.word_off[r];
    const uint32_t* nsrc = reads.nplane ? reads.nplane + reads.word_off[r] : nullptr;
    const int p0 = start[s], L = len[s];
    const int nw = (int)(word_off[s + 1] - word_off[s]);
    const int w0 = p0 >> 4; const uint32_t sh = (uint32_t)(p0 & 15) << 1;
    for (int j = lane; j < nw; j += SP_WAVE) {
        uint32_t v = 0, nv = 0;
// ... 95 lines not shown
    SP_HIP_CHECK(ctx, hipGetLastError());
    if (n && hpc) std::memcpy(h_hlen.data(), h_hl, sizeof(int32_t) * n);
    *seg = sp_seqset();
    seg->ctx = ctx; seg->n = n; seg->has_n = reads->has_n; seg->d_words = d_seg; seg->d_nplane = d_segn; seg->d_word_off = d_woff; seg->d_len = d_len; seg->max_len = max_len;
    seg->h_len = len; seg->h_word_off = h_woff;
    if (hpc) {
        *hpc = *seg;
        hpc->d_words = d_hpc; hpc->d_nplane = d_hpcn; hpc->d_len = d_hlen; hpc->h_len = h_hlen;
    }
    return SP_OK;
}

static int32_t hla_solve_units(sp_ctx* ctx, const sp_hla_db* db, uint32_t n_genes, const uint32_t* genes, const uint32_t* unit_sample,
                               const uint32_t* read_sample, const sp_seqset* reads,
                               const sp_hla_realign* realign, const sp_hla_call_config* cfgs, sp_hla_call* calls,
                               char* cons, uint32_t cap, uint8_t* is_cons1_out, bool clear_is_cons1 = true) {
    if (is_cons1_out && clear_is_cons1) std::memset(is_cons1_out, 0, reads->n);
    HostMarks hm(ctx);
    struct Gene { uint32_t first = 0, n = 0; int is_dual = 0, pass = 0, hemi = 0, used_dna = 0; int32_t c1 = 0, c2 = 0; double maf = 0, cdf = 0; };
    std::vector<Gene> G(n_genes);
    std::vector<uint32_t> sel;
    for (uint32_t k = 0; k < n_genes; ++k) {
        sp_hla_call& call = calls[k];
        std::memset(&call, 0, sizeof call);
        call.allele1 = call.allele2 = call.typed1 = call.typed2 = -1;
        cons[(size_t)(2 * k) * cap] = cons[(size_t)(2 * k + 1) * cap] = '\0';
        G[k].first = (uint32_t)sel.size();
        for (uint32_t r = 0; r < reads->n; ++r)
            if (realign[r].status == 0 && realign[r].gene == (int32_t)genes[k] && (!read_sample || read_sample[r] == unit_sample[k])) sel.push_back(r);
        G[k].n = (uint32_t)sel.size() - G[k].first;
        call.n_reads = (int32_t)G[k].n;
        if (G[k].n == 0) call.status = 1;
    }
    const uint32_t n = (uint32_t)sel.size();
    if (n == 0) return SP_OK;
    SP_HIP_CHECK(ctx, hipSetDevice(ctx->device));

    std::vector<int32_t> h_start(n), h_len(n);
    int32_t max_len = 0;
    for (uint32_t i = 0; i < n; ++i) {
        const sp_hla_realign& q = realign[sel[i]];
        h_start[i] = q.seg_start; h_len[i] = q.seg_end - q.seg_start;
        max_len = std::max(max_len, h_len[i]);
    }
    sp_seqset seg, hpc;
    hm.mark("host:hla_select");
    {
        const int32_t e = sp_make_segments(ctx, reads, sel, h_start, h_len, "hc", &seg, &hpc);
        if (e != SP_OK) return e;
    }
    hm.mark("host:hla_segments");

    const int half_window = 200;
    const uint32_t ccap = (uint32_t)max_len + 512 + 400 + 1;
    std::vector<uint32_t> ident(n);
    for (uint32_t i = 0; i < n; ++i) ident[i] = i;
    std::vector<int32_t> off(n), sc1(n), sc2(n);
    std::vector<uint8_t> is1(n);
    std::vector<char> text((size_t)2 * n_genes * ccap);
    auto cons_config = [&](uint32_t k, int dual) {
        sp_cons_config cc{};
        cc.min_count = cfgs[k].min_consensus_count; cc.min_af = cfgs[k].min_consensus_fraction; cc.dual_max_ed_delta = cfgs[k].dual_max_ed_delta;
        cc.allow_early_termination = 1; cc.allow_dual = dual; cc.offset_window = 400; cc.offset_compare_length = 50;
        return cc;
    };
    auto set_offsets = [&](uint32_t k, bool use_hpc, int group) {
        int32_t mn = INT32_MAX;
        for (uint32_t i = G[k].first; i < G[k].first + G[k].n; ++i) if (group < 0 || is1[i] == group) mn = std::min(mn, use_hpc ? realign[sel[i]].hpc_offset : realign[sel[i]].dna_offset);
        for (uint32_t i = G[k].first; i < G[k].first + G[k].n; ++i) if (group < 0 || is1[i] == group) {
            const int32_t o = use_hpc ? realign[sel[i]].hpc_offset : realign[sel[i]].dna_offset;
            off[i] = o == mn ? -1 : o - mn + half_window;
        }
    };
    auto dual_batch = [&](const std::vector<uint32_t>& which, bool use_hpc) -> int32_t {
        std::vector<sp_cons_problem> P(which.size()); std::vector<sp_cons_output> O(which.size());
        for (size_t x = 0; x < which.size(); ++x) {
            const uint32_t k = which[x];
            set_offsets(k, use_hpc, -1);
            P[x].reads = use_hpc ? &hpc : &seg; P[x].read_idx = ident.data() + G[k].first; P[x].n = G[k].n; P[x].offsets = off.data() + G[k].first; P[x].cfg = cons_config(k, 1);
            std::memset(&O[x], 0, sizeof O[x]);
            O[x].cons1 = text.data() + (size_t)(2 * k) * ccap; O[x].cons2 = text.data() + (size_t)(2 * k + 1) * ccap; O[x].cap = ccap;
            O[x].is_cons1 = is1.data() + G[k].first; O[x].score1 = sc1.data() + G[k].first; O[x].score2 = sc2.data() + G[k].first;
        }
        const int32_t rc = sp_consensus_dual_batch(ctx, (uint32_t)P.size(), P.data(), O.data());
        if (rc != SP_OK) return rc;
        for (size_t x = 0; x < which.size(); ++x) {
            Gene& g = G[which[x]];
            g.is_dual = O[x].result.is_dual;
            g.c1 = 0; for (uint32_t i = g.first; i < g.first + g.n; ++i) g.c1 += is1[i];
            g.c2 = (int32_t)g.n - g.c1;
            if (!g.is_dual) { g.pass = 0; g.maf = g.cdf = 0.0; }
            else g.pass = sp_hla_is_passing_dual((uint64_t)g.c1, (uint64_t)g.c2, cfgs[which[x]].min_consensus_fraction, cfgs[which[x]].expected_maf, cfgs[which[x]].min_cdf, &g.maf, &g.cdf);
        }
        return SP_OK;
    };
    std::vector<uint32_t> todo;
    for (uint32_t k = 0; k < n_genes; ++k) if (G[k].n) todo.push_back(k);
    hm.mark("host:hla_setup");
    int32_t rc = dual_batch(todo, true);
    if (rc != SP_OK) return rc;
    hm.mark("host:hla_dual_hpc");
    std::vector<uint32_t> retry;
    for (uint32_t k : todo) if (!G[k].pass) retry.push_back(k);
    if (!retry.empty()) {
        rc = dual_batch(retry, false);
        if (rc != SP_OK) return rc;
        for (uint32_t k : retry) G[k].used_dna = 1;
    }
    hm.mark("host:hla_dual_dna");
    for (uint32_t k : todo) if (cfgs[k].absent_capable) {
        Gene& g = G[k];
        std::vector<int64_t> s1(g.n), s2(g.n);
        for (uint32_t i = 0; i < g.n; ++i) { s1[i] = sc1[g.first + i]; s2[i] = sc2[g.first + i]; }
        double hc = 0, dc = 0;
        g.hemi = sp_hla_is_hemizygous_better(s1.data(), s2.data(), is1.data() + g.first, g.n, g.is_dual, (uint64_t)cfgs[k].dual_max_ed_delta, cfgs[k].normalized_coverage, &hc, &dc);
        if (g.hemi) { g.is_dual = 0; std::fill(is1.begin() + g.first, is1.begin() + g.first + g.n, (uint8_t)1); }
    }
    struct Grp { uint32_t k; int which; size_t at, n; };
    std::vector<Grp> groups; std::vector<uint32_t> gidx; std::vector<int32_t> goff;
    for (uint32_t k : todo) for (int which = 1; which >= (G[k].is_dual ? 0 : 1); --which) {
        set_offsets(k, false, which);
        Grp g{ k, which, gidx.size(), 0 };
        for (uint32_t i = G[k].first; i < G[k].first + G[k].n; ++i) if (is1[i] == which) { gidx.push_back(i); goff.push_back(off[i]); }
        g.n = gidx.size() - g.at;
        if (g.n) groups.push_back(g);
    }
    {
        std::vector<sp_cons_problem> P(groups.size()); std::vector<sp_cons_output> O(groups.size());
        std::vector<uint8_t> gis(gidx.size()); std::vector<int32_t> gs1(gidx.size()), gs2(gidx.size());
        std::vector<char> spare((size_t)groups.size() * ccap);
        for (size_t x = 0; x < groups.size(); ++x) {
            const Grp& g = groups[x];
            P[x].reads = &seg; P[x].read_idx = gidx.data() + g.at; P[x].n = (uint32_t)g.n; P[x].offsets = goff.data() + g.at; P[x].cfg = cons_config(g.k, 0);
            std::memset(&O[x], 0, sizeof O[x]);
            O[x].cons1 = text.data() + (size_t)(2 * g.k + (g.which ? 0 : 1)) * ccap; O[x].cons2 = spare.data() + x * ccap; O[x].cap = ccap;
            O[x].is_cons1 = gis.data() + g.at; O[x].score1 = gs1.data() + g.at; O[x].score2 = gs2.data() + g.at;
        }
        for (uint32_t k : todo) text[(size_t)(2 * k) * ccap] = text[(size_t)(2 * k + 1) * ccap] = '\0';
        rc = sp_consensus_batch(ctx, (uint32_t)P.size(), P.data(), O.data());
        if (rc != SP_OK && rc != SP_ERR_CAPACITY) return rc;
        for (size_t x = 0; x < groups.size(); ++x) if (O[x].status != SP_OK) O[x].cons1[0] = '\0';
    }
    hm.mark("host:hla_groups");
    std::vector<uint32_t> tg; std::vector<const char*> tp; std::vector<uint32_t> tl; std::vector<std::pair<uint32_t, int>> tw;
    for (uint32_t k : todo) {
        const Gene& g = G[k];
        const char* t1 = text.data() + (size_t)(2 * k) * ccap; const char* t2 = text.data() + (size_t)(2 * k + 1) * ccap;
        const size_t l1 = std::strlen(t1), l2 = g.is_dual ? std::strlen(t2) : 0;
        if (l1 + 1 > cap || l2 + 1 > cap) return sp_fail(ctx, SP_ERR_CAPACITY, "sp_hla_diplotype_genes: consensus buffer too small");
        std::memcpy(cons + (size_t)(2 * k) * cap, t1, l1 + 1); calls[k].cons1_len = (int32_t)l1;
        tg.push_back(genes[k]); tp.push_back(cons + (size_t)(2 * k) * cap); tl.push_back((uint32_t)l1); tw.push_back({ k, 0 });
        if (g.is_dual) {
            std::memcpy(cons + (size_t)(2 * k + 1) * cap, t2, l2 + 1); calls[k].cons2_len = (int32_t)l2;
            tg.push_back(genes[k]); tp.push_back(cons + (size_t)(2 * k + 1) * cap); tl.push_back((uint32_t)l2); tw.push_back({ k, 1 });
        }
    }
    for (int combo = 0; combo < 4; ++combo) {
        const int rd = combo & 1, dc = combo >> 1;
        std::vector<uint32_t> g2; std::vector<const char*> p2; std::vector<uint32_t> l2v; std::vector<size_t> at;
        for (size_t x = 0; x < tw.size(); ++x) if ((cfgs[tw[x].first].require_dna != 0) == rd && (cfgs[tw[x].first].disable_cdna != 0) == dc) { g2.push_back(tg[x]); p2.push_back(tp[x]); l2v.push_back(tl[x]); at.push_back(x); }
        if (g2.empty()) continue;
        std::vector<sp_hla_best> tb(g2.size());
        rc = sp_hla_type_consensus_batch(ctx, db, (uint32_t)g2.size(), g2.data(), p2.data(), l2v.data(), rd, dc, tb.data());
        if (rc != SP_OK) return rc;
        for (size_t y = 0; y < at.size(); ++y) (tw[at[y]].second ? calls[tw[at[y]].first].typed2 : calls[tw[at[y]].first].typed1) = tb[y].best_allele;
    }
    hm.mark("host:hla_typing");
    for (uint32_t k : todo) {
        Gene& g = G[k]; sp_hla_call& call = calls[k];
        call.is_dual = g.is_dual; call.is_hemizygous = g.hemi; call.counts1 = g.c1; call.counts2 = g.c2; call.maf = g.maf; call.cdf = g.cdf; call.used_dna_dual = g.used_dna;
        if (g.is_dual) {
            call.dual_passed = g.pass;
            if (g.pass) { call.allele1 = call.typed1; call.allele2 = call.typed2; }
            else if (g.c1 > g.c2) call.allele1 = call.allele2 = call.typed1;
            else call.allele1 = call.allele2 = call.typed2;
        } else {
            call.dual_passed = 0;
            call.allele1 = call.allele2 = call.typed1;
            if (g.hemi) call.allele1 = -2;
        }
        if (is_cons1_out) for (uint32_t i = g.first; i < g.first + g.n; ++i) is_cons1_out[sel[i]] = is1[i];
    }
    return SP_OK;
}

#ifndef SP_HLA_SPLIT_MIN_READS
#define SP_HLA_SPLIT_MIN_READS 1000
#endif

static int32_t hla_solve_side_by_side(sp_ctx* ctx, const sp_hla_db* db, uint32_t n_units, const uint32_t* genes, const uint32_t* unit_sample,
                                      const uint32_t* read_sample, const sp_seqset* reads, const sp_hla_realign* realign, const sp_hla_call_config* cfgs,
                                      sp_hla_call* calls, char* cons, uint32_t cap, uint8_t* is_cons1_out) {
    HostScope whole(ctx, "host:hla_genes_total");
    uint64_t n_realigned = 0;
    for (uint32_t r = 0; r < reads->n; ++r) n_realigned += realign[r].status == 0;
    int n_parts = (ctx->split_genes && n_realigned >= SP_HLA_SPLIT_MIN_READS) ? (int)std::min<uint32_t>(n_units, (uint32_t)ctx->split_streams) : 1;
    sp_ctx* on[4] = { ctx, nullptr, nullptr, nullptr };
    for (int x = 1; x < n_parts; ++x) { on[x] = sp_ctx_helper(ctx, x - 1); if (!on[x]) { n_parts = x; break; } }
    if (n_parts < 2) return hla_solve_units(ctx, db, n_units, genes, unit_sample, read_sample, reads, realign, cfgs, calls, cons, cap, is_cons1_out);
    if (is_cons1_out) std::memset(is_cons1_out, 0, reads->n);
    struct Part { std::vector<uint32_t> at, genes, samples; std::vector<sp_hla_call_config> cfgs; std::vector<sp_hla_call> calls; std::vector<char> cons; int32_t rc = SP_OK; };
    Part part[4];
    for (uint32_t k = 0; k < n_units; ++k) { Part& q = part[k % (uint32_t)n_parts]; q.at.push_back(k); q.genes.push_back(genes[k]); if (unit_sample) q.samples.push_back(unit_sample[k]); q.cfgs.push_back(cfgs[k]); }
    for (int x = 0; x < n_parts; ++x) { part[x].calls.resize(part[x].at.size()); part[x].cons.assign((size_t)2 * part[x].at.size() * cap, '\0'); }
    auto solve = [&](sp_ctx* c, Part& q) {
        (void)hipSetDevice(c->device);
        try {
            q.rc = hla_solve_units(c, db, (uint32_t)q.at.size(), q.genes.data(), unit_sample ? q.samples.data() : nullptr, read_sample, reads, realign, q.cfgs.data(), q.calls.data(),
                                   q.cons.data(), cap, is_cons1_out, false);
        } catch (const std::bad_alloc&) { q.rc = SP_ERR_OUT_OF_MEMORY; c->err = "sp_hla_diplotype: out of host memory"; }
        catch (const std::exception& e) { q.rc = SP_ERR_INVALID_ARG; c->err = std::string("sp_hla_diplotype: ") + e.what(); }
    };
    HostMarks hm(ctx);
    std::thread beside[4]; bool started[4] = { false, false, false, false };
    for (int x = 1; x < n_parts; ++x) {
        try { beside[x] = std::thread([&, x]() { solve(on[x], part[x]); }); started[x] = true; }
        catch (const std::system_error&) { }
    }
    hm.mark("host:hla_split_spawn");
    solve(ctx, part[0]);
    hm.mark("host:hla_split_own");
    for (int x = 1; x < n_parts; ++x) { if (started[x]) beside[x].join(); else solve(ctx, part[x]); }
// ... 61 lines not shown
```

### pb-starphase_amd/csrc/sp_internal.h

```cpp
#pragma once
#include <hip/hip_runtime.h>
#include <stdint.h>
#include <string>
#include <vector>
#include <chrono>
#include <set>
#include <mutex>
#include <map>
#include "../../include/starphase_hip.h"

#define SP_NEG        (-(1 << 28))
#define SP_SEQ_PAD_WORDS 512
#define SP_LDS_TAIL    288
#define SP_WAVE       64
#define SP_MAXOCC     4
#define SP_CELL_NONE  0xFFFFFFFFu
#define SP_PEAK_SPREAD   48
#define SP_PEAK_SUPPRESS 128

struct SeqSetView {
    const uint32_t* words;
    const uint32_t* nplane;
    const uint64_t* word_off;
    const int32_t*  len;
    uint32_t n;
};

struct KmerIndexView {
    const uint32_t* code;
    const int32_t*  pos;
    const uint64_t* off;
};

struct sp_seqset {
    sp_ctx* ctx = nullptr;
    uint32_t n = 0;
    bool has_n = false;
    std::vector<int32_t>  h_len;
    std::vector<uint64_t> h_word_off;
    std::vector<uint32_t> h_words;
    uint32_t* d_words = nullptr;
    uint32_t* d_nplane = nullptr;
    uint64_t* d_word_off = nullptr;
    int32_t*  d_len = nullptr;
    int32_t   max_len = 0;
    uint32_t  n_skipped = 0;
    struct sp_upload* up = nullptr;
    int32_t up_rc = 0; std::string up_err;
    bool has_index = false;
    uint32_t* d_kcode = nullptr; int32_t* d_kpos = nullptr; uint64_t* d_koff = nullptr;
    SeqSetView view() const { return SeqSetView{d_words, d_nplane, d_word_off, d_len, n}; }
    KmerIndexView kview() const { return KmerIndexView{d_kcode, d_kpos, d_koff}; }
};

struct ProfileEntry { double ms = 0; uint64_t launches = 0; uint64_t cells = 0; };

struct sp_ctx {
    int device = 0;
    hipStream_t stream = nullptr;
    bool own_stream = false;
    std::string err;
    bool profiling = true;
    hipEvent_t ev0 = nullptr, ev1 = nullptr;
    std::map<std::string, ProfileEntry> prof;
    struct PendingProf { hipEvent_t e0, e1; const char* name; uint64_t cells; };
    std::vector<PendingProf> prof_pending;
    std::vector<hipEvent_t> prof_free;
    void* scratch = nullptr; size_t scratch_bytes = 0;
    std::map<std::string, std::pair<void*, size_t>> pool;
    uint64_t pool_allocs = 0;
    std::map<std::string, std::pair<void*, size_t>> host_pool;
    std::multimap<size_t, void*> dev_cache; std::map<void*, size_t> dev_cap; size_t dev_cache_bytes = 0; std::mutex dev_cache_mu;
    std::set<sp_seqset*> live_sets;
    int num_cus = 256;
    int hw_queues = 4; bool hw_queues_by_library = false; std::string warning;
    bool split_genes = true;
    int split_streams = 3;
    bool cons_retry_ladder = false;
    hipStream_t copy_stream = nullptr;
    hipStream_t ctl_stream = nullptr;
    hipEvent_t ev_fork = nullptr, ev_join = nullptr;
    int k1_best_n = 5;
    int profile_rescore_counts = 0;
    int mm2_rescore = 1;
    int k8_persistent = 2;
    int hw_queues_effective = 0;
    int k8_side_orders = 1;
    int k8_compound = 1;
    int k8_side_max_blocks = 4096;
    int k8_persist_backoff = 0;
    int k8_persist_failures = 0;
    sp_seqset* uploading = nullptr;
    int k5_block_pairs = 4096;
    int cyp_cohort_min_group = 12;
    int cyp_cohort_streams = 8;
    sp_ctx* helper[7] = { nullptr, nullptr, nullptr, nullptr, nullptr, nullptr, nullptr };
};

struct CellDesc {
    uint32_t a, b;
    int32_t  diag;
    int32_t  max_ed;
    int32_t  b_lo, b_hi;
};

struct K2Dict {
    bool built = false, failed = false;
    uint32_t* d_ids = nullptr;
    uint64_t* d_id_off = nullptr;
    uint32_t* d_code = nullptr;
    uint32_t* d_dict_off = nullptr;
    std::vector<uint32_t> dict_off;
    uint32_t n_dict = 0, max_dict = 0;
};
void* sp_dev_alloc(sp_ctx* ctx, size_t bytes);
void sp_dev_release(sp_ctx* ctx, void* p);
int  sp_k2_dict_build(sp_ctx* ctx, const sp_seqset* set, const uint32_t* d_gene_of, uint32_t n_genes, K2Dict* out);
void sp_k2_dict_free(K2Dict* d);

struct K1Seed;
struct K1SeedDebug {
    uint32_t read;
    int32_t* chains; uint32_t chain_cap; uint32_t* n_chains;
    sp_k1_seed_hit* hits; uint32_t* n_hits;
    uint64_t* counters;
};
int  sp_k1_seed_build(sp_ctx* ctx, const sp_seqset* alleles, K1Seed** out);
void sp_k1_seed_free(K1Seed* s);
void sp_k1_seed_stats(const K1Seed* s, int64_t out[4]);
int  sp_k1_seed_sketch(sp_ctx* ctx, const sp_seqset* set, uint32_t idx, uint64_t* hash, int32_t* end_pos, uint8_t* strand, uint32_t cap, uint32_t* n_out);
int  sp_k1_seed_map(sp_ctx* ctx, const K1Seed* idx, const sp_seqset* alleles, const sp_seqset* reads, int best_n, int32_t* d_best, sp_k1_seed_info* d_info,
                    sp_aln* d_win_aln, sp_affine_aln* d_win_af, const K1SeedDebug* dbg, sp_hla_rev_hit* d_rev = nullptr);

sp_ctx* sp_ctx_helper(sp_ctx* ctx, int i = 0);
void sp_profile_merge(sp_ctx* into, sp_ctx* from);
int sp_launch_anchor(sp_ctx* ctx, const sp_seqset* A, const sp_seqset* B,
                     const uint32_t* d_a_idx, const uint32_t* d_b_idx, uint64_t n_pairs,
                     int32_t* d_diag, int32_t* d_votes, int topk = 1, const char* prof_name = "anchor", uint32_t a_period = 1);
int sp_launch_cells(sp_ctx* ctx, const sp_seqset* A, const sp_seqset* B,
                    const CellDesc* d_cells, uint64_t n_cells,
                    sp_aln* d_out, uint32_t* d_events, uint32_t events_stride, const char* prof_name, int retry_wide = 0);

int sp_launch_affine(sp_ctx* ctx, const sp_seqset* A, const sp_seqset* B, const void* d_pairs , uint64_t n_pairs, const sp_affine_opts& o, int band,
                     sp_affine_aln* d_out, const char* prof_name, const uint32_t* d_n_live = nullptr, const void* d_wins = nullptr, const void* d_mids = nullptr);
int sp_rescore_mappings(sp_ctx* ctx, const sp_seqset* Aw, const sp_seqset* Bw, const CellDesc* d_cells, const sp_aln* d_ref, uint64_t n, bool target_is_a,
                        const sp_affine_opts& o, int band, sp_affine_aln* d_out, const char* prefix, uint32_t stride, int trace_retry_wide = 0, const sp_aln* d_tr_in = nullptr, const uint32_t* d_ev_in = nullptr, int ends_only = 0, int windows = -1, void* d_audit = nullptr);
int sp_launch_affine_map(sp_ctx* ctx, const sp_seqset* A, const sp_seqset* B, const void* d_pairs , uint64_t n_pairs, const sp_affine_opts& o, sp_affine_aln* d_out,
                         uint32_t* d_n_cigar, uint64_t* d_op_off, uint32_t* d_ops, uint64_t ops_cap, unsigned long long* d_cursor, const char* prof_name);
constexpr uint32_t SP_ANCHOR_SKIP = 0xFFFFFFFFu;
int sp_launch_cells_wide(sp_ctx* ctx, const sp_seqset* A, const sp_seqset* B, const CellDesc* d_cells, uint64_t n_cells, sp_aln* d_out);
int sp_launch_pack_on(hipStream_t stream, int num_cus, int format, const void* d_src, const uint64_t* d_off, const uint64_t* d_word_off, const int32_t* d_len, uint32_t n,
                      uint32_t* d_words, uint32_t* d_nplane, uint32_t* d_flag);
int sp_launch_pack(sp_ctx* ctx, const char* d_ascii, const uint64_t* d_off, const uint64_t* d_word_off, const int32_t* d_len, uint32_t n,
                   uint32_t* d_words, uint32_t* d_nplane, uint32_t* d_flag);
int sp_make_segments(sp_ctx* ctx, const sp_seqset* reads, const std::vector<uint32_t>& idx, const std::vector<int32_t>& start,
                     const std::vector<int32_t>& len, const char* prefix, sp_seqset* seg, sp_seqset* hpc);
int sp_seqset_make_small(sp_ctx* ctx, const char* prefix, const char* bases, const uint64_t* offsets, uint32_t n, bool with_index, sp_seqset* out);
int sp_seqset_fetch_host(sp_ctx* ctx, sp_seqset* s);
std::string sp_seqset_decode(sp_ctx* ctx, const sp_seqset* s, uint32_t i);
enum { SPC_K1_ACTIVE = 0, SPC_K1_EXECUTED, SPC_K1_RESUMED, SPC_K1_BYTES, SPC_CONS_LAUNCHES, SPC_CONS_COLUMNS, SPC_N = 16 };
unsigned long long* sp_counters(sp_ctx* ctx);
void* sp_scratch(sp_ctx* ctx, size_t bytes);
void* sp_pool(sp_ctx* ctx, const char* name, size_t bytes);
size_t sp_pool_bytes(const sp_ctx* ctx, const char* name);
void* sp_host_pool(sp_ctx* ctx, const char* name, size_t bytes);
int   sp_fail(sp_ctx* ctx, int code, const std::string& msg);
#define SP_HIP_CHECK(ctx, expr) do { hipError_t _e = (expr); if (_e != hipSuccess) \
    return sp_fail((ctx), SP_ERR_HIP, std::string(#expr) + ": " + hipGetErrorString(_e)); } while (0)

void sp_profile_flush(sp_ctx* ctx);
struct HostMarks {
    sp_ctx* ctx; std::chrono::steady_clock::time_point t;
    explicit HostMarks(sp_ctx* c) : ctx(c), t(std::chrono::steady_clock::now()) {}
    void mark(const char* name) { const auto now = std::chrono::steady_clock::now(); if (ctx->profiling) { auto& e = ctx->prof[name]; e.ms += std::chrono::duration<double, std::milli>(now - t).count(); e.launches += 1; } t = now; }
};
struct HostScope {
    sp_ctx* ctx; const char* name; std::chrono::steady_clock::time_point t0;
    HostScope(sp_ctx* c, const char* n) : ctx(c), name(n), t0(std::chrono::steady_clock::now()) {}
    ~HostScope() { if (ctx->profiling) { auto& e = ctx->prof[name]; e.ms += std::chrono::duration<double, std::milli>(std::chrono::steady_clock::now() - t0).count(); e.launches += 1; } }
};
struct ProfScope {
    sp_ctx* ctx; const char* name; uint64_t cells; hipEvent_t e0 = nullptr, e1 = nullptr;
    ProfScope(sp_ctx* c, const char* n, uint64_t cells_) : ctx(c), name(n), cells(cells_) {
        if (!(ctx->profiling && name)) return;
        auto take = [&]() { hipEvent_t e = nullptr; if (!ctx->prof_free.empty()) { e = ctx->prof_free.back(); ctx->prof_free.pop_back(); } else if (hipEventCreate(&e) != hipSuccess) e = nullptr; return e; };
        e0 = take(); e1 = take();
        if (e0 && e1) hipEventRecord(e0, ctx->stream);
    }
    ~ProfScope() {
        if (!(e0 && e1)) { if (e0) ctx->prof_free.push_back(e0); if (e1) ctx->prof_free.push_back(e1); return; }
        hipEventRecord(e1, ctx->stream);
        ctx->prof_pending.push_back({e0, e1, name, cells});
        if (ctx->prof_pending.size() >= 2048) sp_profile_flush(ctx);
    }
};


int32_t spi_gene_entry_extras(const sp_database* db, const sp_variant_gene* g, std::string* reference_allele, bool* has_sv, std::string* sv_chrom);
std::string spi_hla_allele_fwd(sp_ctx* ctx, const sp_hla_db* db, uint32_t a);
int spi_hla_gene_fwd(const sp_hla_db* db, uint32_t gene);
int32_t spi_hla_map_type_batch(sp_ctx* ctx, const sp_hla_db* db, uint32_t n, const uint32_t* genes, const char* const* consensus_fwd, const uint32_t* consensus_len,
                               int32_t require_dna, int32_t disable_cdna, sp_hla_map** out, std::vector<uint32_t>* item_of);
int32_t spi_cyp_diplotype_mappings(sp_ctx* ctx, const sp_cyp_problem* pr, const sp_seqset* reads, sp_cyp_call* call, char* consensus, uint32_t cons_cap,
                                   sp_cyp_region_variants* region_variants, std::vector<sp_cyp_read_mapping>* mappings);
int32_t spi_cyp_diplotype_cohort_mappings(sp_ctx* ctx, const sp_cyp_problem* pr, uint32_t n_samples, const sp_seqset* const* reads, sp_cyp_call* calls,
                                          char* consensus, uint32_t cons_cap, sp_cyp_region_variants* region_variants,
                                          std::vector<sp_cyp_read_mapping>* mappings, int32_t* sample_rc);
```

Before: 359,500 reads/s.

## Add a per-device tick server that merges consensus step launches across contexts

```diff
diff --git a/pb-starphase_amd/csrc/sp_api.hip b/pb-starphase_amd/csrc/sp_api.hip
--- a/pb-starphase_amd/csrc/sp_api.hip
+++ b/pb-starphase_amd/csrc/sp_api.hip
@@ -52,6 +52,7 @@
     ctx->hw_queues_effective = effective.load();
     { const char* kc = std::getenv("SP_K8_COMPOUND"); if (kc && *kc) ctx->k8_compound = std::atoi(kc); }
     { const char* ks = std::getenv("SP_K8_SIDE_ORDERS"); if (ks && *ks) ctx->k8_side_orders = std::max(0, std::min(3, std::atoi(ks))); }
+    { const char* kt = std::getenv("SP_K8_TICKS"); if (kt && *kt) { const int v = std::atoi(kt); if (v >= 0 && v <= 2) ctx->k8_ticks = v; } }
     { const char* kp = std::getenv("SP_K8_PERSISTENT"); if (kp && *kp) ctx->k8_persistent = std::atoi(kp); }
     if (effective.load() == 0)
         ctx->warning = "the HIP runtime was initialised before the library's first context and GPU_MAX_HW_QUEUES was not set: the process's streams share the runtime's 4 hardware queues; "
@@ -65,6 +66,7 @@
         ctx->own_stream = true;
     }
     if (hipEventCreate(&ctx->ev0) != hipSuccess || hipEventCreate(&ctx->ev1) != hipSuccess) { delete ctx; return SP_ERR_HIP; }
+    sp_k8_ticks_ctx_created(device);
     *out = ctx;
     return SP_OK;
 }
@@ -101,6 +103,7 @@
     if (ctx->ev0) hipEventDestroy(ctx->ev0);
     if (ctx->ev1) hipEventDestroy(ctx->ev1);
     if (ctx->own_stream && ctx->stream) hipStreamDestroy(ctx->stream);
+    sp_k8_ticks_ctx_destroyed(ctx->device);
     delete ctx;
 }
 
@@ -108,7 +111,7 @@
 sp_ctx* sp_ctx_helper(sp_ctx* ctx, int i) {
     if (i < 0 || i > 6) return nullptr;
     if (!ctx->helper[i] && sp_ctx_create(ctx->device, nullptr, &ctx->helper[i]) != SP_OK) ctx->helper[i] = nullptr;
-    if (ctx->helper[i]) { ctx->helper[i]->profiling = ctx->profiling; ctx->helper[i]->k5_block_pairs = ctx->k5_block_pairs; ctx->helper[i]->k8_persistent = ctx->k8_persistent; ctx->helper[i]->k8_side_orders = ctx->k8_side_orders; ctx->helper[i]->k8_compound = ctx->k8_compound; ctx->helper[i]->k8_side_max_blocks = ctx->k8_side_max_blocks; ctx->helper[i]->mm2_rescore = ctx->mm2_rescore; ctx->helper[i]->profile_rescore_counts = ctx->profile_rescore_counts; ctx->helper[i]->k1_best_n = ctx->k1_best_n; }
+    if (ctx->helper[i]) { ctx->helper[i]->profiling = ctx->profiling; ctx->helper[i]->k5_block_pairs = ctx->k5_block_pairs; ctx->helper[i]->k8_persistent = ctx->k8_persistent; ctx->helper[i]->k8_ticks = ctx->k8_ticks; ctx->helper[i]->k8_side_orders = ctx->k8_side_orders; ctx->helper[i]->k8_compound = ctx->k8_compound; ctx->helper[i]->k8_side_max_blocks = ctx->k8_side_max_blocks; ctx->helper[i]->mm2_rescore = ctx->mm2_rescore; ctx->helper[i]->profile_rescore_counts = ctx->profile_rescore_counts; ctx->helper[i]->k1_best_n = ctx->k1_best_n; }
     return ctx->helper[i];
 }
 void sp_profile_merge(sp_ctx* into, sp_ctx* from) {
@@ -196,6 +199,7 @@
     if (std::strcmp(name, "k8_side_orders") == 0) { if (value < 0 || value > 3) return sp_fail(ctx, SP_ERR_INVALID_ARG, "sp_ctx_set_option: k8_side_orders is 0 .. 3"); ctx->k8_side_orders = (int)value; for (sp_ctx* h : ctx->helper) if (h) h->k8_side_orders = ctx->k8_side_orders; return SP_OK; }
     if (std::strcmp(name, "k8_compound") == 0) { ctx->k8_compound = (int)value; for (sp_ctx* h : ctx->helper) if (h) h->k8_compound = ctx->k8_compound; return SP_OK; }
     if (std::strcmp(name, "k8_side_max_blocks") == 0) { if (value < 0) return sp_fail(ctx, SP_ERR_INVALID_ARG, "sp_ctx_set_option: k8_side_max_blocks >= 0"); ctx->k8_side_max_blocks = (int)value; for (sp_ctx* h : ctx->helper) if (h) h->k8_side_max_blocks = ctx->k8_side_max_blocks; return SP_OK; }
+    if (std::strcmp(name, "k8_ticks") == 0) { if (value < 0 || value > 2) return sp_fail(ctx, SP_ERR_INVALID_ARG, "sp_ctx_set_option: k8_ticks is 0 (a launch chain per context), 1 (the device's tick server) or 2 (the library decides)"); ctx->k8_ticks = (int)value; for (sp_ctx* h : ctx->helper) if (h) h->k8_ticks = ctx->k8_ticks; return SP_OK; }
     if (std::strcmp(name, "k8_persistent") == 0) { if (value < 0 || value > 2) return sp_fail(ctx, SP_ERR_INVALID_ARG, "sp_ctx_set_option: k8_persistent is 0 (never), 1 (whenever a batch fits) or 2 (the library decides)"); ctx->k8_persistent = (int)value; ctx->k8_persist_backoff = 0; ctx->k8_persist_failures = 0; for (sp_ctx* h : ctx->helper) if (h) h->k8_persistent = ctx->k8_persistent; return SP_OK; }
     if (std::strcmp(name, "cons_retry_ladder") == 0) { ctx->cons_retry_ladder = value != 0; for (sp_ctx* h : ctx->helper) if (h) h->cons_retry_ladder = ctx->cons_retry_ladder; return SP_OK; }
     if (std::strcmp(name, "k5_block_pairs") == 0) { if (value < 0 || value > (1 << 20)) return sp_fail(ctx, SP_ERR_INVALID_ARG, "sp_ctx_set_option: k5_block_pairs is 0..1048576"); ctx->k5_block_pairs = (int)value; for (sp_ctx* h : ctx->helper) if (h) h->k5_block_pairs = ctx->k5_block_pairs; return SP_OK; }
diff --git a/pb-starphase_amd/csrc/sp_consensus.hip b/pb-starphase_amd/csrc/sp_consensus.hip
--- a/pb-starphase_amd/csrc/sp_consensus.hip
+++ b/pb-starphase_amd/csrc/sp_consensus.hip
@@ -1,11 +1,15 @@
 #include "sp_internal.h"
+#include "sp_k8_ticks.h"
 #include <atomic>
 #include <cstdlib>
+#include <thread>
 #include "sp_wfa.hip.h"
 #include <algorithm>
 #include <cstddef>
 #include <cstring>
 #include <map>
+#include <mutex>
+#include <new>
 #include <string>
 
 namespace {
@@ -595,6 +599,9 @@
 #define SP_K8_DIRECT_BLOCKS (680 * 8 / SP_K8_WAVES)
 #endif
 constexpr int DIRECT_BLOCKS = SP_K8_DIRECT_BLOCKS;
+#ifndef SP_K8_TICKS_RULE
+#define SP_K8_TICKS_RULE 0
+#endif
 constexpr int32_t SP_K8_AGAIN = -777;
 constexpr int PERSIST_BLOCKS = 128 * 8 / CWAVES;
 
@@ -619,7 +626,7 @@
 }
 
 template <int MAXP>
-__device__ __forceinline__ void cons_step_body(const ConsBatchT<MAXP>& B, const int wrow) {
+__device__ __forceinline__ void cons_step_body(const ConsBatchT<MAXP>& B, const int wrow, const int bx) {
     __shared__ unsigned long long lv[2][CW + 1];
     __shared__ uint32_t le[2][CW + 1];
     __shared__ unsigned long long ll[2][CW];
@@ -629,7 +636,7 @@
     __shared__ uint32_t cpk[2][(CWIN + CW) / 16 + 2];
     __shared__ ActScratch act[CWAVES];
     __shared__ CWork wk_s;
-    const int pi = block_problem<MAXP>(B);
+    const int pi = block_problem<MAXP>(B, bx);
     const ConsParams P = B.p[pi];
     const bool coh = B.sync != nullptr;
     if (coh) {
@@ -671,7 +678,7 @@
     __syncthreads();
     const size_t plane = (size_t)B.total;
     for (int rr = 0; rr < P.rpw; ++rr) {
-        const int r = (((int)blockIdx.x - P.first_block) * CWAVES + wave) * P.rpw + rr;
+        const int r = ((bx - P.first_block) * CWAVES + wave) * P.rpw + rr;
         if (r >= P.n) break;
         const size_t g = (size_t)P.first + r;
 #ifdef SP_K8_TIMING
@@ -1126,18 +1133,18 @@
     }
     for (int x = threadIdx.x; x < 2 * uw.used; x += blockDim.x) {
         const int i = x / uw.used, e = i * (CW + 1) + x % uw.used;
-        B.PV[(size_t)blockIdx.x * 2 * (CW + 1) + e] = (&lv[0][0])[e];
-        B.PE[(size_t)blockIdx.x * 2 * (CW + 1) + e] = (&le[0][0])[e];
-    }
-    if (uw.has_la) for (int x = threadIdx.x; x < 2 * CW; x += blockDim.x) B.PL[(size_t)blockIdx.x * 2 * CW + x] = (&ll[0][0])[x];
-    for (int x = threadIdx.x; x < uw.used; x += blockDim.x) { B.PC[(size_t)blockIdx.x * (CW + 1) + x] = lc[x]; B.PR[(size_t)blockIdx.x * (CW + 1) + x] = lr[x]; }
+        B.PV[(size_t)bx * 2 * (CW + 1) + e] = (&lv[0][0])[e];
+        B.PE[(size_t)bx * 2 * (CW + 1) + e] = (&le[0][0])[e];
+    }
+    if (uw.has_la) for (int x = threadIdx.x; x < 2 * CW; x += blockDim.x) B.PL[(size_t)bx * 2 * CW + x] = (&ll[0][0])[x];
+    for (int x = threadIdx.x; x < uw.used; x += blockDim.x) { B.PC[(size_t)bx * (CW + 1) + x] = lc[x]; B.PR[(size_t)bx * (CW + 1) + x] = lr[x]; }
     if (B.step_t && threadIdx.x == 0) atomicMax(&B.step_t[2 * pi + 1], (unsigned long long)wall_clock64());
 }
 
 template <int MAXP>
-__global__ void __launch_bounds__(CWAVES * SP_WAVE, SP_K8_MIN_WAVES) cons_step_kernel(ConsBatchT<MAXP> B) { cons_step_body<MAXP>(B, (int)blockIdx.y); }
+__global__ void __launch_bounds__(CWAVES * SP_WAVE, SP_K8_MIN_WAVES) cons_step_kernel(ConsBatchT<MAXP> B) { cons_step_body<MAXP>(B, (int)blockIdx.y, (int)blockIdx.x); }
 template <int MAXP>
-__global__ void __launch_bounds__(CWAVES * SP_WAVE, 2) cons_step_wide_kernel(ConsBatchT<MAXP> B) { cons_step_body<MAXP>(B, (int)blockIdx.y); }
+__global__ void __launch_bounds__(CWAVES * SP_WAVE, 2) cons_step_wide_kernel(ConsBatchT<MAXP> B) { cons_step_body<MAXP>(B, (int)blockIdx.y, (int)blockIdx.x); }
 
 template <int MAXP>
 __global__ void __launch_bounds__(512) cons_reduce_kernel(ConsBatchT<MAXP> B) {
@@ -1213,7 +1220,7 @@
 }
 
 template <int MAXP>
-__device__ __forceinline__ void cons_control_body(const ConsBatchT<MAXP>& B) {
+__device__ __forceinline__ void cons_control_body(const ConsBatchT<MAXP>& B, const int pi) {
     extern __shared__ uint8_t proc[];
     __shared__ uint32_t acc[QE];
     uint32_t (*sv)[CW + 1][5] = reinterpret_cast<uint32_t (*)[CW + 1][5]>(acc);
@@ -1226,7 +1233,6 @@
     struct KidCopy { int from, T, n, nk, dual; int8_t node[4], b0[4], b1[4], sp[4]; uint8_t spec[2][CW]; };
     static_assert(KID_LA_KIDS <= 4, "KidCopy");
     __shared__ KidCopy kcopy[NWORK];
-    const int pi = blockIdx.x;
     const ConsParams P = B.p[pi];
     const int tid = threadIdx.x;
     const bool coh = B.sync != nullptr;
@@ -1929,7 +1935,29 @@
 }
 
 template <int MAXP>
-__global__ void __launch_bounds__(1024) cons_control_kernel(ConsBatchT<MAXP> B) { cons_control_body<MAXP>(B); }
+__global__ void __launch_bounds__(1024) cons_control_kernel(ConsBatchT<MAXP> B) { cons_control_body<MAXP>(B, (int)blockIdx.x); }
+
+constexpr int TICK_MAX = sp_k8_ticks::MAX_LIVE;
+struct TickEntry { const ConsBatchT<0>* B; int first_block, first_prob; };
+struct TickList { TickEntry e[TICK_MAX]; int n; };
+
+__device__ __forceinline__ void tick_step(const TickList& L) {
+    const ConsBatchT<0>* bp = L.e[0].B; int first = 0;
+#pragma unroll
+    for (int i = 1; i < TICK_MAX; ++i) if (i < L.n && (int)blockIdx.x >= L.e[i].first_block) { bp = L.e[i].B; first = L.e[i].first_block; }
+    const ConsBatchT<0> B = *bp;
+    if ((int)blockIdx.y > B.nside) return;
+    cons_step_body<0>(B, (int)blockIdx.y, (int)blockIdx.x - first);
+}
+__global__ void __launch_bounds__(CWAVES * SP_WAVE, SP_K8_MIN_WAVES) cons_step_tick_kernel(TickList L) { tick_step(L); }
+__global__ void __launch_bounds__(CWAVES * SP_WAVE, 2) cons_step_tick_wide_kernel(TickList L) { tick_step(L); }
+__global__ void __launch_bounds__(1024) cons_control_tick_kernel(TickList L) {
+    const ConsBatchT<0>* bp = L.e[0].B; int first = 0;
+#pragma unroll
+    for (int i = 1; i < TICK_MAX; ++i) if (i < L.n && (int)blockIdx.x >= L.e[i].first_prob) { bp = L.e[i].B; first = L.e[i].first_prob; }
+    const ConsBatchT<0> B = *bp;
+    cons_control_body<0>(B, (int)blockIdx.x - first);
+}
 
 constexpr long long PERSIST_TIMEOUT = 400000000ll;
 constexpr double PERSIST_READY_S = 0.5;
@@ -1955,7 +1983,7 @@
         __syncthreads();
         if (!go_on) break;
         if (coh_load(&B.p[pi].work->done)) break;
-        cons_step_body<MAXP>(B, 0);
+        cons_step_body<MAXP>(B, 0, (int)blockIdx.x);
         asm volatile("s_waitcnt vmcnt(0)" ::: "memory");
         __syncthreads();
         if (threadIdx.x == 0) __hip_atomic_fetch_add(sy + 1, 1u, __ATOMIC_RELAXED, __HIP_MEMORY_SCOPE_AGENT);
@@ -1977,7 +2005,7 @@
         __syncthreads();
         if (!go_on) break;
         __builtin_amdgcn_fence(__ATOMIC_ACQUIRE, "agent");
-        cons_control_body<MAXP>(B);
+        cons_control_body<MAXP>(B, pi);
         asm volatile("s_waitcnt vmcnt(0)" ::: "memory");
         __syncthreads();
         const bool done = coh_load(&B.p[pi].work->done) != 0;
@@ -2098,8 +2126,75 @@
     ~PersistLease() { give_back(); }
 };
 
+namespace {
+struct TickServer {
+    int device = 0, num_cus = 256;
+    hipStream_t stream = nullptr;
+    sp_k8_ticks::Table table;
+    std::thread thread;
+    size_t lds_set = 0;
+    static bool ok(hipError_t e, std::string& err) { if (e != hipSuccess) err = hipGetErrorString(e); return e == hipSuccess; }
+    bool wait_for(void* ready, std::string& err) { return ok(hipStreamWaitEvent(stream, (hipEvent_t)ready, 0), err); }
+    bool record(void* done, std::string& err) { return ok(hipEventRecord((hipEvent_t)done, stream), err); }
+    sp_k8_ticks::Query query(std::string& err) {
+        const hipError_t q = hipStreamQuery(stream);
+        if (q == hipSuccess) return sp_k8_ticks::Q_IDLE;
+        if (q == hipErrorNotReady) return sp_k8_ticks::Q_BUSY;
+        err = hipGetErrorString(q); return sp_k8_ticks::Q_ERROR;
+    }
+    void drain() { (void)hipStreamSynchronize(stream); (void)hipGetLastError(); }
+    bool launch(const std::vector<sp_k8_ticks::Batch*>& live, std::string& err) {
+        TickList L; std::memset(&L, 0, sizeof L);
+        int nb = 0, np = 0, nside = 0; size_t lds = 0;
+        for (const sp_k8_ticks::Batch* b : live) {
+            TickEntry& e = L.e[L.n++];
+            e.B = (const ConsBatchT<0>*)b->desc; e.first_block = nb; e.first_prob = np;
+            nb += b->n_blocks; np += b->n_prob; nside = std::max(nside, b->nside); lds = std::max(lds, b->proc_lds);
+        }
+        if (lds > lds_set) { if (!ok(hipFuncSetAttribute((const void*)cons_control_tick_kernel, hipFuncAttributeMaxDynamicSharedMemorySize, (int)lds), err)) return false; lds_set = lds; }
+        const dim3 grid((uint32_t)nb, (uint32_t)(1 + nside)), block(CWAVES * SP_WAVE);
+        if (nb <= (num_cus + num_cus / 4) * (8 / CWAVES)) hipLaunchKernelGGL(cons_step_tick_wide_kernel, grid, block, 0, stream, L);
+        else hipLaunchKernelGGL(cons_step_tick_kernel, grid, block, 0, stream, L);
+        hipLaunchKernelGGL(cons_control_tick_kernel, dim3((uint32_t)np), dim3(1024), lds, stream, L);
+        return ok(hipGetLastError(), err);
+    }
+    void run() { (void)hipSetDevice(device); sp_k8_ticks::serve(table, *this); }
+};
+static_assert(sp_k8_ticks::ERR_DEVICE == SP_ERR_HIP && sp_k8_ticks::AHEAD == 3, "sp_k8_ticks.h");
+std::mutex tick_mu;
+TickServer* tick_servers[64];
+int tick_contexts[64];
+TickServer* tick_server(sp_ctx* ctx) {
+    std::lock_guard<std::mutex> g(tick_mu);
+    TickServer*& s = tick_servers[ctx->device & 63];
+    if (!s) {
+        TickServer* n = new (std::nothrow) TickServer();
+        if (!n) return nullptr;
+        n->device = ctx->device; n->num_cus = ctx->num_cus;
+        if (hipStreamCreateWithFlags(&n->stream, hipStreamNonBlocking) != hipSuccess) { delete n; return nullptr; }
+        try { n->thread = std::thread(&TickServer::run, n); } catch (...) { (void)hipStreamDestroy(n->stream); delete n; return nullptr; }
+        s = n;
+    }
+    return s;
+}
+}
+void sp_k8_ticks_ctx_created(int device) { std::lock_guard<std::mutex> g(tick_mu); ++tick_contexts[device & 63]; }
+void sp_k8_ticks_ctx_destroyed(int device) {
+    TickServer* s = nullptr;
+    {
+        std::lock_guard<std::mutex> g(tick_mu);
+        if (--tick_contexts[device & 63] > 0) return;
+        s = tick_servers[device & 63]; tick_servers[device & 63] = nullptr;
+    }
+    if (!s) return;
+    s->table.stop();
+    s->thread.join();
+    (void)hipStreamSynchronize(s->stream); (void)hipStreamDestroy(s->stream);
+    delete s;
+}
+
 template <int MAXP>
-static int32_t run_chunk(sp_ctx* ctx, uint32_t n_prob, const sp_cons_problem* probs, sp_cons_output* outs) {
+static int32_t run_chunk(sp_ctx* ctx, uint32_t n_prob, const sp_cons_problem* probs, sp_cons_output* outs, const bool ticks = false) {
     hipStream_t st = ctx->stream;
     HostMarks hm(ctx);
     ConsBatchT<MAXP> B; std::memset(&B, 0, sizeof B);
@@ -2138,7 +2233,7 @@
     uint64_t footprint = 2 * (uint64_t)n_prob;
     for (uint32_t p = 0; p < n_prob; ++p) footprint += ((probs[p].read_idx ? probs[p].n : probs[p].reads->n) + CWAVES - 1) / CWAVES;
     const bool light = footprint <= (uint64_t)PERSIST_LIGHT;
-    const bool persist_wanted = ctx->k8_persistent == 1 || (ctx->k8_persistent == 2 && n_prob <= 8 && ctx->hw_queues_effective >= 16 && ctx->k8_persist_failures < 3 &&
+    const bool persist_wanted = ctx->k8_persistent == 1 || (!(ticks && ctx->k8_ticks == 1) && ctx->k8_persistent == 2 && n_prob <= 8 && ctx->hw_queues_effective >= 16 && ctx->k8_persist_failures < 3 &&
                                                             !in_flight.recent_overlap && light);
     if (ctx->k8_persist_backoff > 0) --ctx->k8_persist_backoff;
     else if (persist_wanted && n_prob > 0) {
@@ -2374,6 +2469,31 @@
                 persist_rpw = 0;
             }
         }
+        if constexpr (MAXP == 0) if (ticks && !finished && !persist_rpw && !need_reduce) {
+            {
+                hipFuncAttributes fa;
+                SP_HIP_CHECK(ctx, hipFuncGetAttributes(&fa, (const void*)cons_control_tick_kernel));
+                if (fa.sharedSizeBytes + proc_lds > 160 * 1024) return sp_fail(ctx, SP_ERR_TOO_LONG, "sp_consensus: cap must stay below ~65,000");
+            }
+            if (!ctx->ev_fork && (hipEventCreateWithFlags(&ctx->ev_fork, hipEventDisableTiming) != hipSuccess || hipEventCreateWithFlags(&ctx->ev_join, hipEventDisableTiming) != hipSuccess))
+                return sp_fail(ctx, SP_ERR_HIP, "sp_consensus: events");
+            ConsBatchT<0>* d_desc = (ConsBatchT<0>*)sp_pool(ctx, "cons_desc", sizeof B); ConsBatchT<0>* h_desc = (ConsBatchT<0>*)sp_host_pool(ctx, "cons_desc", sizeof B);
+            if (!d_desc || !h_desc) return sp_fail(ctx, SP_ERR_OUT_OF_MEMORY, "sp_consensus descriptor");
+            TickServer* srv = tick_server(ctx);
+            if (!srv) return sp_fail(ctx, SP_ERR_HIP, "sp_consensus: tick server");
+            *h_desc = B;
+            SP_HIP_CHECK(ctx, hipMemcpyAsync(d_desc, h_desc, sizeof B, hipMemcpyHostToDevice, st));
+            SP_HIP_CHECK(ctx, hipEventRecord(ctx->ev_fork, st));
+            sp_k8_ticks::Batch tb;
+            tb.desc = d_desc; tb.n_blocks = n_blocks; tb.n_prob = (int)n_prob; tb.nside = B.nside; tb.proc_lds = proc_lds;
+            tb.ready = ctx->ev_fork; tb.done = ctx->ev_join; tb.prog = h_prog; tb.limit = limit;
+            srv->table.submit(&tb);
+            srv->table.wait_back(&tb);
+            if (tb.status != 0) return sp_fail(ctx, tb.status, tb.error);
+            SP_HIP_CHECK(ctx, hipStreamWaitEvent(st, ctx->ev_join, 0));
+            pairs = tb.ticks; finished = true;
+            ctx->prof["cons_tick_batches"].cells += 1; ctx->prof["cons_tick_joins_running"].cells += tb.joined_running ? 1 : 0; ctx->prof["cons_tick_launches"].cells += tb.ticks;
+        }
         while (!finished) {
             const auto tl0 = std::chrono::steady_clock::now();
             if (one_round) hipLaunchKernelGGL(cons_step_wide_kernel<MAXP>, grid, block, 0, st, B);
@@ -2518,7 +2638,15 @@
     const uint32_t big = 4096;
     for (uint32_t at = 0; at < n_prob; at += big) {
         const uint32_t k = std::min<uint32_t>(big, n_prob - at);
-        auto run = [&]() { return k <= 4 ? run_chunk<4>(ctx, k, probs + at, outs + at) : k <= 8 ? run_chunk<8>(ctx, k, probs + at, outs + at)
+        static const int tick_rule = [] { const char* e = std::getenv("SP_K8_TICKS_RULE"); return e && *e ? std::atoi(e) : SP_K8_TICKS_RULE; }();
+        bool ticks = ctx->k8_persistent != 1 && (ctx->k8_ticks == 1 || (ctx->k8_ticks == 2 && (tick_rule == 2 || (tick_rule == 1 && !ctx->k8_caller_hla))));
+        for (uint32_t p = at; ticks && p < at + k; ++p) {
+            const uint32_t n = probs[p].read_idx ? probs[p].n : probs[p].reads->n;
+            const uint32_t per_block = (uint32_t)CWAVES * (n > 65536 ? 4u : n > 32768 ? 2u : 1u);
+            if ((n + per_block - 1) / per_block > (uint32_t)DIRECT_BLOCKS) ticks = false;
+        }
+        auto run = [&]() { return ticks ? run_chunk<0>(ctx, k, probs + at, outs + at, true)
+                                  : k <= 4 ? run_chunk<4>(ctx, k, probs + at, outs + at) : k <= 8 ? run_chunk<8>(ctx, k, probs + at, outs + at)
                                   : k <= CMAXP ? run_chunk<CMAXP>(ctx, k, probs + at, outs + at) : run_chunk<0>(ctx, k, probs + at, outs + at); };
         int32_t e = run();
         if (e == SP_K8_AGAIN) e = run();
diff --git a/pb-starphase_amd/csrc/sp_hla_call.hip b/pb-starphase_amd/csrc/sp_hla_call.hip
--- a/pb-starphase_amd/csrc/sp_hla_call.hip
+++ b/pb-starphase_amd/csrc/sp_hla_call.hip
@@ -201,7 +201,9 @@
             O[x].cons1 = text.data() + (size_t)(2 * k) * ccap; O[x].cons2 = text.data() + (size_t)(2 * k + 1) * ccap; O[x].cap = ccap;
             O[x].is_cons1 = is1.data() + G[k].first; O[x].score1 = sc1.data() + G[k].first; O[x].score2 = sc2.data() + G[k].first;
         }
+        ctx->k8_caller_hla = true;
         const int32_t rc = sp_consensus_dual_batch(ctx, (uint32_t)P.size(), P.data(), O.data());
+        ctx->k8_caller_hla = false;
         if (rc != SP_OK) return rc;
         for (size_t x = 0; x < which.size(); ++x) {
             Gene& g = G[which[x]];
@@ -256,7 +258,9 @@
             O[x].is_cons1 = gis.data() + g.at; O[x].score1 = gs1.data() + g.at; O[x].score2 = gs2.data() + g.at;
         }
         for (uint32_t k : todo) text[(size_t)(2 * k) * ccap] = text[(size_t)(2 * k + 1) * ccap] = '\0';
+        ctx->k8_caller_hla = true;
         rc = sp_consensus_batch(ctx, (uint32_t)P.size(), P.data(), O.data());
+        ctx->k8_caller_hla = false;
         if (rc != SP_OK && rc != SP_ERR_CAPACITY) return rc;
         for (size_t x = 0; x < groups.size(); ++x) if (O[x].status != SP_OK) O[x].cons1[0] = '\0';
     }
diff --git a/pb-starphase_amd/csrc/sp_internal.h b/pb-starphase_amd/csrc/sp_internal.h
--- a/pb-starphase_amd/csrc/sp_internal.h
+++ b/pb-starphase_amd/csrc/sp_internal.h
@@ -85,6 +85,8 @@
     int mm2_rescore = 1;
     int k8_persistent = 2;
     int hw_queues_effective = 0;
+    int k8_ticks = 2;
+    bool k8_caller_hla = false;
     int k8_side_orders = 1;
     int k8_compound = 1;
     int k8_side_max_blocks = 4096;
@@ -132,6 +134,8 @@
 int  sp_k1_seed_map(sp_ctx* ctx, const K1Seed* idx, const sp_seqset* alleles, const sp_seqset* reads, int best_n, int32_t* d_best, sp_k1_seed_info* d_info,
                     sp_aln* d_win_aln, sp_affine_aln* d_win_af, const K1SeedDebug* dbg, sp_hla_rev_hit* d_rev = nullptr);
 
+void sp_k8_ticks_ctx_created(int device);
+void sp_k8_ticks_ctx_destroyed(int device);
 sp_ctx* sp_ctx_helper(sp_ctx* ctx, int i = 0);
 void sp_profile_merge(sp_ctx* into, sp_ctx* from);
 int sp_launch_anchor(sp_ctx* ctx, const sp_seqset* A, const sp_seqset* B,
diff --git a/pb-starphase_amd/csrc/sp_k8_ticks.h b/pb-starphase_amd/csrc/sp_k8_ticks.h
--- /dev/null
+++ b/pb-starphase_amd/csrc/sp_k8_ticks.h
@@ -0,0 +1,140 @@
+#pragma once
+#include <atomic>
+#include <condition_variable>
+#include <cstdint>
+#include <deque>
+#include <mutex>
+#include <string>
+#include <vector>
+#if defined(__x86_64__) || defined(__i386__)
+#include <immintrin.h>
+#endif
+
+namespace sp_k8_ticks {
+
+constexpr int MAX_LIVE = 16;
+constexpr uint32_t AHEAD = 3;
+constexpr int32_t ERR_DEVICE = 3;
+
+struct Batch {
+    const void* desc = nullptr;
+    int n_blocks = 0, n_prob = 0, nside = 0;
+    size_t proc_lds = 0;
+    void* ready = nullptr;
+    void* done = nullptr;
+    const volatile uint32_t* prog = nullptr;
+    uint64_t limit = 0;
+    int32_t status = 0; std::string error;
+    uint64_t ticks = 0;
+    uint64_t last_tick = 0;
+    bool joined_running = false;
+    int state = 0;
+
+    static uint32_t word(const volatile uint32_t* w) { return __atomic_load_n(w, __ATOMIC_ACQUIRE); }
+    bool ended() const { for (int p = 0; p < n_prob; ++p) if (!word(prog + 2 * p + 1)) return false; return true; }
+    uint32_t slowest() const { uint32_t s = 0xFFFFFFFFu; for (int p = 0; p < n_prob; ++p) if (!word(prog + 2 * p + 1)) { const uint32_t v = word(prog + 2 * p); s = v < s ? v : s; } return s; }
+};
+
+class Table {
+public:
+    void submit(Batch* b) {
+        { std::lock_guard<std::mutex> g(mu_); b->state = 1; queued_.push_back(b); n_queued_.store(queued_.size(), std::memory_order_release); }
+        cv_server_.notify_one();
+    }
+    void wait_back(Batch* b) { std::unique_lock<std::mutex> g(mu_); cv_back_.wait(g, [&] { return b->state == 3; }); }
+    void stop() { { std::lock_guard<std::mutex> g(mu_); stop_ = true; } cv_server_.notify_one(); }
+
+    bool wait_work() {
+        if (!live_.empty() || n_queued_.load(std::memory_order_acquire)) return true;
+        std::unique_lock<std::mutex> g(mu_);
+        cv_server_.wait(g, [&] { return stop_ || !queued_.empty(); });
+        return !queued_.empty();
+    }
+    void pick_up(std::vector<Batch*>& joined) {
+        if (!n_queued_.load(std::memory_order_acquire) || (int)live_.size() >= MAX_LIVE) return;
+        std::lock_guard<std::mutex> g(mu_);
+        while (!queued_.empty() && (int)live_.size() < MAX_LIVE) {
+            Batch* b = queued_.front(); queued_.pop_front();
+            b->state = 2; b->joined_running = !live_.empty();
+            live_.push_back(b); joined.push_back(b);
+        }
+        n_queued_.store(queued_.size(), std::memory_order_release);
+    }
+    const std::vector<Batch*>& live() const { return live_; }
+    uint64_t tick_no() const { return tick_no_; }
+    void tick_launched() { ++tick_no_; for (Batch* b : live_) { ++b->ticks; b->last_tick = tick_no_; } }
+    template <class F> void hand_back_if(F leaves) {
+        std::vector<Batch*> out;
+        for (size_t i = 0; i < live_.size();) if (leaves(live_[i])) { out.push_back(live_[i]); live_.erase(live_.begin() + (long)i); } else ++i;
+        if (out.empty()) return;
+        { std::lock_guard<std::mutex> g(mu_); for (Batch* b : out) b->state = 3; }
+        cv_back_.notify_all();
+    }
+    void fail_all(int32_t code, const std::string& text) { hand_back_if([&](Batch* b) { b->status = code; b->error = text; return true; }); }
+
+private:
+    std::mutex mu_;
+    std::condition_variable cv_server_, cv_back_;
+    std::deque<Batch*> queued_;
+    std::atomic<size_t> n_queued_{0};
+    std::vector<Batch*> live_;
+    uint64_t tick_no_ = 0;
+    bool stop_ = false;
+};
+
+enum Query { Q_IDLE, Q_BUSY, Q_ERROR };
+
+inline void cpu_pause() {
+#if defined(__x86_64__) || defined(__i386__)
+    _mm_pause();
+#endif
+}
+
+template <class Dev>
+void serve(Table& T, Dev& dev, const uint64_t guard_mask = 0xFFFFF) {
+    std::vector<Batch*> joined;
+    uint64_t spins = 0;
+    std::string err;
+    auto fail = [&](const std::string& text) { dev.drain(); T.fail_all(ERR_DEVICE, text); spins = 0; };
+    while (T.wait_work()) {
+        joined.clear();
+        T.pick_up(joined);
+        bool ok = true;
+        for (Batch* b : joined) if (!dev.wait_for(b->ready, err)) { ok = false; break; }
+        if (!ok) { fail("sp_consensus: " + err); continue; }
+        bool rec_failed = false;
+        T.hand_back_if([&](Batch* b) {
+            if (rec_failed) return false;
+            const bool ended = b->ended();
+            if (!ended && b->ticks < b->limit) return false;
+            if (!dev.record(b->done, err)) { rec_failed = true; return false; }
+            if (!ended) { b->status = ERR_DEVICE; b->error = "sp_consensus: the search did not finish"; }
+            return true;
+        });
+        if (rec_failed) { fail("sp_consensus: " + err); continue; }
+        if (T.live().empty()) continue;
+        bool within = true;
+        for (Batch* b : T.live()) if (!b->ended() && b->ticks - (uint64_t)b->slowest() > AHEAD) { within = false; break; }
+        if (within) {
+            bool any_open = false;
+            for (Batch* b : T.live()) any_open = any_open || !b->ended();
+            if (!any_open) continue;
+            if (!dev.launch(T.live(), err)) { fail("sp_consensus: " + err); continue; }
+            T.tick_launched();
+            spins = 0;
+            continue;
+        }
+        cpu_pause();
+        if ((++spins & guard_mask) == 0) {
+            const Query q = dev.query(err);
+            if (q == Q_ERROR) { fail("sp_consensus: " + err); continue; }
+            if (q == Q_IDLE) {
+                bool ended = false, behind = false;
+                for (Batch* b : T.live()) { if (b->ended()) ended = true; else if (b->ticks - (uint64_t)b->slowest() > AHEAD) behind = true; }
+                if (behind && !ended) fail("sp_consensus: the device stopped reporting progress");
+            }
+        }
+    }
+}
+
+}
```

After: 344,500 reads/s. -4.2%, worse.
